# Linyou/Ced-NeRF

Hardware: AMD Instinct MI355X
Metric: samples_per_sec (render_image_test, 800x800 D-NeRF lego-shaped synthetic) (higher is better)
Workload: dtype f32 (MLP GEMMs: split-fp16 MFMA, 22-bit operands, fp32 accumulate)

## Files before the change

### ced_nerf_amd/_lib.py

```python
from __future__ import annotations

import ctypes as C
import os
import subprocess
from typing import List, Optional

_PKG = os.path.dirname(os.path.abspath(__file__))
_ROOT = os.path.dirname(_PKG)
LIB_PATH = os.environ.get("CED_NERF_LIB", os.path.join(_PKG, "libcednerf_hip.so"))
SOURCES = ["runtime.hip", "march.hip", "composite.hip", "field.hip", "hash.hip", "field_half.hip", "field_mixed.hip", "field_move.hip", "field_jacobian.hip", "field_density_gradient.hip", "field_time_max.hip", "field_level_set.hip", "surface.hip", "frame_loop.hip", "frame.hip", "image.hip", "march_all.hip", "occgrid.hip",
           "raygen.hip", "wgrad.hip", "pixels.hip", "accel.hip", "linear.hip", "mlp.hip", "train_glue.hip", "losses.hip",
           "metrics.hip", "train_batch.hip", "importance.hip", "bake.hip", "mesh.hip"]
MLP_F32, MLP_F16X2, MLP_F16, MLP_F32_HEAD16X2 = 0, 1, 2, 3
MLP_PRECISIONS = {"f32": MLP_F32, "f16x2": MLP_F16X2, "f16": MLP_F16, "f32+h16x2": MLP_F32_HEAD16X2}
HIPCC_FLAGS = ["--offload-arch=gfx950", "-O3", "-ffp-contract=off", "-fno-slp-vectorize", "-fPIC", "-shared", "-std=c++17"]
PER_SOURCE_FLAGS = {"field_half.hip": ["-mllvm", "-amdgpu-sched-strategy=max-memory-clause"]}
MAX_LEVELS = 16


class HashDesc(C.Structure):
    _fields_ = [
        ("n_levels", C.c_int32), ("table_dtype", C.c_int32), ("temporal", C.c_int32), ("reserved", C.c_int32),
        ("scale", C.c_float * MAX_LEVELS), ("res", C.c_uint32 * MAX_LEVELS), ("offset", C.c_uint32 * MAX_LEVELS),
        ("size", C.c_uint32 * MAX_LEVELS), ("hashed", C.c_uint32 * MAX_LEVELS),
        ("table", C.c_void_p), ("total_entries", C.c_uint64),
    ]


class FieldDesc(C.Structure):
    _fields_ = [
        ("aabb", C.c_float * 6), ("moving_step", C.c_float), ("use_div_offsets", C.c_int32),
        ("time_mode", C.c_int32), ("mlp_precision", C.c_int32), ("max_workgroups", C.c_int32),
        ("packed_weights", C.c_void_p), ("packed_floats", C.c_uint64),
        ("hash", HashDesc),
    ]


class FrameTrace(C.Structure):
    _fields_ = [
        ("capacity", C.c_int32), ("n_iters", C.c_int32),
        ("field_begin", C.POINTER(C.c_void_p)), ("field_end", C.POINTER(C.c_void_p)),
        ("iter_alive", C.POINTER(C.c_int64)), ("iter_n_samples", C.POINTER(C.c_int64)),
        ("iter_samples", C.POINTER(C.c_int64)), ("field_stamps", C.c_void_p),
    ]


EXCHANGE_FN = C.CFUNCTYPE(C.c_int, C.c_void_p, C.c_void_p, C.c_int32, C.c_int32, C.c_void_p)


class ShardExchange(C.Structure):
    _fields_ = [
        ("global_rays_per_frame", C.c_int64), ("local_rays", C.c_void_p), ("counts", C.c_void_p),
        ("reduce", EXCHANGE_FN), ("user", C.c_void_p),
    ]


_vp, _i64, _i32, _f = C.c_void_p, C.c_int64, C.c_int32, C.c_float

PROTOTYPES = {
    "ced_version": (C.c_int, []),
    "ced_last_error_string": (C.c_char_p, []),
    "ced_set_option": (C.c_int, [C.c_char_p, C.c_int]),
    "ced_packed_weight_floats": (_i64, [C.c_int, C.c_int]),
    "ced_pack_field_weights": (C.c_int, [C.c_int, C.c_int] + [_vp] * 10),
    "ced_packed_weight_words": (_i64, [C.c_int, C.c_int, C.c_int]),
    "ced_pack_field_weights_half": (C.c_int, [C.c_int, C.c_int, C.c_int] + [_vp] * 10),
    "ced_pack_field_weights_half_for": (C.c_int, [C.c_int] * 5 + [_vp] * 10),
    "ced_pack_field_weights_mixed": (C.c_int, [C.c_int, C.c_int] + [_vp] * 10),
    "ced_ray_aabb_intersect": (C.c_int, [_i64, _vp, _vp, _i32, _vp, _f, _f, _f, _vp, _vp, _vp, _vp]),
    "ced_sort_intersections": (C.c_int, [_i64, _i32, _vp, _vp, _vp, _vp, _vp]),
    "ced_traverse_grids": (C.c_int, [_i64, _vp, _vp, _vp, _i32, _i32, _vp, _vp, _vp, _f, _f, _i32, _vp, _vp, _vp, _vp,
                                     _i32, _vp, _vp, _vp, _vp, _vp, _vp, _vp, _vp]),
    "ced_host_skip_march": (_f, [_f, _f, _f, _f]),
    "ced_occupancy_accel_bytes": (_i64, [_i32, _i32]),
    "ced_build_occupancy_accel": (C.c_int, [_vp, _i32, _i32, _vp, _i64, _vp]),
    "ced_host_build_occupancy_accel": (C.c_int, [_vp, _i32, _i32, _vp]),
    "ced_host_count_steps": (_i32, [C.POINTER(C.c_float), _f, _f, _i32, C.POINTER(C.c_float)]),
    "ced_host_march_frame": (C.c_int, [_i64, _vp, _vp, _vp, _i32, _i32, _vp, _vp, _f, _f, _f, _i32, _vp, _vp, _vp, _vp, _i32, _i32,
                                       _i32, _vp, _vp, _vp, _vp]),
    "ced_hash_encode": (C.c_int, [C.POINTER(HashDesc), _i64, _vp, _vp, _vp, _vp]),
    "ced_hash_encode_backward": (C.c_int, [C.POINTER(HashDesc), _i64, _vp, _vp, _vp, _vp, _i32, _vp]),
    "ced_hash_encode_backward_temporal": (C.c_int, [C.POINTER(HashDesc), _i64, _vp, _vp, _vp, _vp, _vp]),
    "ced_field_forward": (C.c_int, [C.POINTER(FieldDesc), _i64, _vp, _vp, _vp, _vp, _vp, _vp, _vp]),
    "ced_field_forward_rays": (C.c_int, [C.POINTER(FieldDesc), _i64, _vp, _vp, _vp, _vp, _vp, _vp, _vp, _i32, _i32,
                                         _vp, _vp, _vp]),
    "ced_field_move": (C.c_int, [C.POINTER(FieldDesc), _i64, _vp, _vp, _vp, _vp, _vp, _vp, _vp]),
    "ced_field_move_rays": (C.c_int, [C.POINTER(FieldDesc), _i64, _vp, _vp, _vp, _vp, _vp, _vp, _vp, _i32, _vp, _vp, _vp]),
    "ced_field_move_inverse": (C.c_int, [C.POINTER(FieldDesc), _i64, _vp, _vp, _vp, _i32, _f, _vp, _vp, _vp, _vp]),
    "ced_field_track": (C.c_int, [C.POINTER(FieldDesc), _i64, _i64, _vp, _vp, _vp, _i32, _f, _vp, _vp, _vp, _vp]),
    "ced_field_move_jacobian": (C.c_int, [C.POINTER(FieldDesc), _i64, _vp, _vp, _vp, _vp, _vp]),
    "ced_field_density_gradient": (C.c_int, [C.POINTER(FieldDesc), _i64, _vp, _vp, _vp, _vp, _vp, _vp, _vp]),
    "ced_field_density_gradient_rays": (C.c_int, [C.POINTER(FieldDesc), _i64, _vp, _vp, _vp, _vp, _vp, _vp, _vp, _i32, _vp, _vp,
                                                  _vp, _vp, _vp]),
    "ced_field_density_time_max": (C.c_int, [C.POINTER(FieldDesc), _i64, _vp, _i32, _i32, _vp, _vp, _vp]),
    "ced_surface_first_crossing": (C.c_int, [_i64, _vp, _vp, _vp, _vp, _f, _vp, _vp, _vp, _vp]),
    "ced_field_level_set": (C.c_int, [C.POINTER(FieldDesc), _i64, _vp, _vp, _vp, _vp, _vp, _i32, _f, _i32, _f, _vp, _vp, _vp, _vp,
                                      _vp, _vp, _vp]),
    "ced_field_velocity": (C.c_int, [C.POINTER(FieldDesc), _i64, _vp, _vp, _vp, _vp, _vp, _vp]),
    "ced_field_velocity_rays": (C.c_int, [C.POINTER(FieldDesc), _i64, _vp, _vp, _vp, _vp, _vp, _vp, _vp, _i32, _vp, _vp, _vp, _vp]),
    "ced_field_move_inverse_newton": (C.c_int, [C.POINTER(FieldDesc), _i64, _vp, _vp, _vp, _i32, _f, _vp, _vp, _vp, _vp]),
    "ced_field_track_newton": (C.c_int, [C.POINTER(FieldDesc), _i64, _i64, _vp, _vp, _vp, _i32, _f, _vp, _vp, _vp, _vp]),
    "ced_field_rgb": (C.c_int, [C.POINTER(FieldDesc), _i64, _vp, _vp, _i32, _vp, _vp]),
    "ced_field_rgb_bcast": (C.c_int, [C.POINTER(FieldDesc), _i64, _i32, _vp, _vp, _i32, _vp, _vp]),
    "ced_bake_workspace_bytes": (_i64, [_i64]),
    "ced_bake_candidates": (C.c_int, [_i32, C.POINTER(C.c_float), _f, _i64, _i64, _vp, _vp, _i32, _i32, _i64, _vp, _vp, _vp,
                                      _vp, _i64, _vp]),
    "ced_bake_select": (C.c_int, [_i64, _vp, _vp, _vp, _vp, _f, _i64, _vp, _vp, _vp, _vp, _vp, _vp, _i64, _vp]),
    "ced_mesh_workspace_bytes": (_i64, [_i32]),
    "ced_mesh_vertices": (C.c_int, [_i32, C.POINTER(C.c_float), _f, _vp, _f, _i64, _vp, _vp, _vp, _vp, _vp, _i64, _vp]),
    "ced_mesh_faces": (C.c_int, [_i32, _vp, _f, _vp, _i64, _i64, _vp, _vp, _vp, _i64, _vp]),
    "ced_render_weights": (C.c_int, [_i64, _vp, _vp, _vp, _vp, _vp, _vp, _vp, _vp, _vp]),
    "ced_accumulate_along_rays": (C.c_int, [_i64, _vp, _vp, _vp, _i32, _vp, _vp]),
    "ced_reduce_along_rays": (C.c_int, [_i64, _vp, _vp, _i32, _vp, _i32, _i64, _i32, _vp, _vp, _vp]),
    "ced_visibility_mask": (C.c_int, [_i64, _vp, _vp, _vp, _vp, _f, _f, _vp, _vp]),
    "ced_composite_prefix": (C.c_int, [_i64, _vp, _vp, _vp, _vp, _vp, _vp, _vp, _vp, _vp]),
    "ced_composite_backward": (C.c_int, [_i64, _vp, _vp, _vp, _vp, _vp, _vp, _vp, _vp, _vp, _vp, _vp]),
    "ced_distortion_workspace_bytes": (_i64, [_i64, _i64, _i32]),
    "ced_distortion_loss": (C.c_int, [_i64, _i64] + [_vp] * 10),
    "ced_distortion_loss_density": (C.c_int, [_i64, _i64] + [_vp] * 10),
    "ced_ssim_workspace_bytes": (_i64, [_i64, _i64, _i64, _i64, _i32, _i32]),
    "ced_ssim": (C.c_int, [_i64, _i64, _i64, _i64, _vp, C.POINTER(_i64), _vp, C.POINTER(_i64), C.c_double, C.c_double,
                           C.c_double, _i32, C.POINTER(C.c_float), _i32, C.POINTER(C.c_float), _i32, _vp, _vp, _vp, _vp,
                           _vp, _vp]),
    "ced_frame_to_rgb8": (C.c_int, [_i32, _i32, _vp, _i32, _vp, _vp]),
    "ced_flow_to_rgb8": (C.c_int, [_i32, _i32, _vp, _f, _i32, _vp, _vp]),
    "ced_depth_to_u8": (C.c_int, [_i32, _i32, _vp, _i32, _vp, _vp, _vp]),
    "ced_scatter_pixels": (C.c_int, [_i64, _vp, _i32, _vp, _i32, _vp, _i32, _vp, _i64, _vp, _vp, _vp, _vp, _i32, _i32, _vp]),
    "ced_linear": (C.c_int, [_i64, _vp, _i32, _vp, _i32, _i32, _i32, _i32, _i32, _vp, _vp, _vp]),
    "ced_weight_grad_workspace_bytes": (_i64, [_i64, _i32, _i32]),
    "ced_weight_grad": (C.c_int, [_i64, _vp, _i32, _vp, _i32, _vp, _vp, _i64, _vp]),
    "ced_composite_step": (C.c_int, [_i64, _vp, _vp, _vp, _vp, _vp, _vp, _vp, _vp, _f, _i32, _vp, _vp, _vp]),
    "ced_composite_test": (C.c_int, [_i64, _vp, _vp, _vp, _vp, _vp, _vp, _f, _f, _vp, _vp, _vp, _vp]),
    "ced_finalize_pixels": (C.c_int, [_i64, _vp, _vp, _vp, _vp, _vp]),
    "ced_occ_cell_points": (C.c_int, [_i64, _vp, _vp, _i32, C.POINTER(C.c_float), _vp, _vp]),
    "ced_occ_ema_update": (C.c_int, [_i64, _vp, _vp, _f, _f, _vp, _vp, _i64, _vp]),
    "ced_occ_time_slices_workspace_bytes": (_i64, [_i32, _i32, _i32]),
    "ced_occ_time_slices": (C.c_int, [_i64, _vp, _vp, _i32, _f, _f, _i32, _i32, _vp, _i32, _vp, _vp, _i64, _vp]),
    "ced_generate_rays_pinhole": (C.c_int, [_i32, _i32, _f, _f, _f, _f, C.POINTER(C.c_float), _i32, _vp, _vp, _vp, _vp]),
    "ced_generate_rays_hypercam": (C.c_int, [_i32, _i32, C.POINTER(C.c_float), C.POINTER(C.c_float), _f, _f, _f, _f, _f,
                                             C.POINTER(C.c_float), C.POINTER(C.c_float), _vp, _vp, _vp]),
    "ced_sample_training_batch": (C.c_int, [_i32] * 5 + [_vp] * 3 + [_i64, C.c_uint64, _i64, _i32, _i32] + [_vp] * 7),
    "ced_importance_batch_workspace_bytes": (_i64, [_i64, _i64, _i64]),
    "ced_sample_importance_batch": (C.c_int, [_i32] * 5 + [_vp] * 4 + [_i32, _i64, _i64, C.c_uint64, _i64, _i32] + [_vp] * 8
                                    + [_i64, _vp]),
    "ced_temporal_median_u8": (C.c_int, [_i32] * 4 + [_vp] * 3),
    "ced_isg_weights": (C.c_int, [_i32] * 4 + [_vp, _vp, _f, _vp, _vp]),
    "ced_ist_weights": (C.c_int, [_i32] * 4 + [_vp, _f, _i32, _vp, _vp]),
    "ced_render_image_test_workspace_bytes": (_i64, [_i64, _i32, _i32, _f, _i32]),
    "ced_render_image_test": (C.c_int, [C.POINTER(FieldDesc), _i64, _vp, _vp, _vp, _i32, _i32, _vp, _vp, _f, _f, _f, _f, _f,
                                        _i32, _vp, _i32, _vp, _vp, _vp, _vp, _vp, _i64, _vp, C.POINTER(_i64),
                                        C.POINTER(FrameTrace), _vp, _vp]),
    "ced_render_frames_test_workspace_bytes": (_i64, [_i32, _i64, _i32, _i32, _f, _i32]),
    "ced_render_frames_test": (C.c_int, [C.POINTER(FieldDesc), _i32, _i64, _vp, _vp, _vp, _i32, _i32, _vp, _vp, _f, _f, _f, _f,
                                         _f, _i32, _vp, _vp, _vp, _vp, _vp, _vp, _i64, _vp, C.POINTER(_i64),
                                         C.POINTER(FrameTrace), _vp, _vp]),
    "ced_render_frames_test_sharded_workspace_bytes": (_i64, [_i32, _i64, _i64, _i32, _i32, _f, _i32]),
    "ced_render_frames_test_iterations": (_i32, [_f, _i32]),
    "ced_render_frames_test_host_bytes": (_i64, [_f, _i32]),
    "ced_render_frames_test_sharded": (C.c_int, [C.POINTER(FieldDesc), _i32, _i64, _vp, _vp, _vp, _i32, _i32, _vp, _vp, _f, _f, _f,
                                                 _f, _f, _i32, _vp, _vp, _vp, _vp, _vp, _vp, _i64, _vp, C.POINTER(_i64),
                                                 C.POINTER(FrameTrace), _vp, _vp, C.POINTER(ShardExchange)]),
    "ced_wall_clock_khz": (_i64, []),
    "ced_mlp_chain": (C.c_int, [_i64, _i32, _i32, _vp, C.POINTER(_i32), C.POINTER(_vp), C.POINTER(_vp), C.POINTER(_vp), _i32, _vp]),
    "ced_march_all": (C.c_int, [_i64, _vp, _vp, _vp, _i32, _i32, _vp, _vp, _vp, _f, _f, _f, _vp, _vp, _vp, _i32, _vp, _vp, _vp,
                                _vp, _i64, _vp, _vp]),
    "ced_render_image_workspace_bytes": (_i64, [_i64, _i64]),
    "ced_render_image": (C.c_int, [C.POINTER(FieldDesc), _i64, _vp, _vp, _i64, _vp, _vp, _vp, _f, _f, _vp, _i32, _vp, _vp, _vp,
                                   _vp, _vp, _vp, _i64, _vp, C.POINTER(_i64), _vp, _vp]),
    "ced_mlp_backward_dw_workspace_bytes": (_i64, [_i64, _i32, C.POINTER(_i32)]),
    "ced_mlp_backward_dw": (C.c_int, [_i64, _i32, _vp, C.POINTER(_i32), C.POINTER(_vp), C.POINTER(_vp), _vp, _vp, _vp, _i64, _vp]),
    "ced_train_inputs": (C.c_int, [_i64] + [_vp] * 13),
    "ced_train_warp": (C.c_int, [_i64, _vp, _vp, _i32, _i32, _f, C.POINTER(C.c_float), _vp, _vp, _vp, _vp]),
    "ced_train_warp_backward": (C.c_int, [_i64, _vp, _vp, _i32, _i32, _f, C.POINTER(C.c_float), _vp, _vp, _vp, _vp]),
    "ced_train_head_in": (C.c_int, [_i64] + [_vp] * 6),
    "ced_train_head_in_backward": (C.c_int, [_i64] + [_vp] * 6),
    "ced_render_image_gather": (C.c_int, [_i64, _i64, _i64, _vp, _i64, _vp, _i64, _vp, _vp, _vp, _vp, _vp, _vp, _vp, _vp, _vp]),
}


def _includes(path: str, seen=None) -> List[str]:
    import re
    seen = set() if seen is None else seen
    if path in seen or not os.path.exists(path):
        return []
    seen.add(path)
    out = [path]
    for inc in re.findall(r'^\s*#\s*include\s+"([^"]+)"', open(path).read(), flags=re.M):
        out += _includes(os.path.normpath(os.path.join(os.path.dirname(path), inc)), seen)
    return out


def build(force: bool = False, verbose: bool = False, extra_flags: Optional[List[str]] = None) -> str:
    from concurrent.futures import ThreadPoolExecutor
    srcs = [os.path.join(_PKG, "csrc", s) for s in SOURCES]
    hipcc = os.environ.get("HIPCC", "hipcc")
    flags = [f for f in HIPCC_FLAGS if f != "-shared"] + list(extra_flags or [])
    obj_dir = os.path.join(_ROOT, "build", "obj")
    os.makedirs(obj_dir, exist_ok=True)
    stamp = os.path.join(obj_dir, "flags.txt")
    flag_text = " ".join([hipcc] + flags + [f"{k}:{' '.join(v)}" for k, v in sorted(PER_SOURCE_FLAGS.items())])
    if not os.path.exists(stamp) or open(stamp).read() != flag_text:
        force = True
    jobs, objs = [], []
    for src in srcs:
        obj = os.path.join(obj_dir, os.path.basename(src) + ".o")
        objs.append(obj)
        deps = _includes(src)
        if force or not os.path.exists(obj) or any(os.path.getmtime(obj) < os.path.getmtime(d) for d in deps):
            jobs.append([hipcc] + flags + PER_SOURCE_FLAGS.get(os.path.basename(src), []) + ["-c", src, "-o", obj])
    if not jobs and os.path.exists(LIB_PATH) and all(os.path.getmtime(LIB_PATH) >= os.path.getmtime(o) for o in objs):
        return LIB_PATH

    def run(cmd):
        if verbose:
            print(" ".join(cmd), flush=True)
        subprocess.check_call(cmd)

    workers = max(1, min(len(jobs), int(os.environ.get("CED_BUILD_JOBS", str(min(os.cpu_count() or 1, 8))))))
    if jobs:
        with ThreadPoolExecutor(max_workers=workers) as pool:
            list(pool.map(run, jobs))
    run([hipcc, "--offload-arch=gfx950", "-shared", "-fPIC", "-o", LIB_PATH] + objs)
    from . import _k32_gate
    _, bad = _k32_gate.check(LIB_PATH)
    if bad:
        os.remove(LIB_PATH)
        raise RuntimeError("K = 32 residency gate failed (ced_nerf_amd/_k32_gate.py): "
                           + "; ".join(f"{k}: {v}" for k, v in sorted(bad.items())))
    with open(stamp, "w") as f:
        f.write(flag_text)
    return LIB_PATH


_lib: Optional[C.CDLL] = None


def lib() -> C.CDLL:
    global _lib
    if _lib is None:
        if not os.path.exists(LIB_PATH):
            raise RuntimeError(
                f"{LIB_PATH} not found: build the HIP extension first (python -c 'import __graft_entry__ as g; "
                "g.build()'); ced_nerf_amd has no CPU fallback")
        handle = C.CDLL(LIB_PATH)
        for name, (res, args) in PROTOTYPES.items():
            fn = getattr(handle, name)
            fn.restype = res
            fn.argtypes = args
        _lib = handle
        for item in filter(None, os.environ.get("CED_OPTIONS", "").split(",")):
            key, _, value = item.partition("=")
            if handle.ced_set_option(key.strip().encode(), int(value)) != 0:
                raise RuntimeError(f"CED_OPTIONS: {handle.ced_last_error_string().decode()}")
    return _lib


def check(rc: int, what: str = "") -> None:
    if rc != 0:
        msg = lib().ced_last_error_string()
        raise RuntimeError(f"libcednerf_hip {what} failed (code {rc}): {msg.decode() if msg else ''}")


def header_symbols() -> List[str]:
    import re
    text = open(os.path.join(_ROOT, "include", "cednerf_hip.h")).read()
    text = re.sub(r"/\*.*?\*/", "", text, flags=re.S)
    return sorted(set(re.findall(r"\b(ced_[a-z0-9_]+)\s*\(", text)))
```

### ced_nerf_amd/csrc/accel.hip

```cpp
#include <algorithm>
#include <vector>

#include "ced_common.hpp"
#include "march_accel.hpp"

namespace ced {

constexpr int kDistCap = 15;

__global__ __launch_bounds__(64) void brick_any_kernel(const uint8_t *__restrict__ binaries, int res, int nb,
                                                       uint8_t *__restrict__ any)
{
    const int idx = blockIdx.x;
    const int bz = idx % nb, by = (idx / nb) % nb, bx = (idx / (nb * nb)) % nb, lvl = idx / (nb * nb * nb);
    const uint8_t *g = binaries + (size_t)lvl * res * res * res;
    const int x = bx * kBrick + (threadIdx.x >> 3), y = by * kBrick + (threadIdx.x & 7);
    uint8_t acc = 0;
    if (x < res && y < res)
        for (int z = bz * kBrick; z < min((bz + 1) * kBrick, res); ++z) acc |= g[((size_t)x * res + y) * res + z];
    const unsigned long long any_lane = __ballot(acc != 0);
    if (threadIdx.x == 0) any[idx] = any_lane ? 0 : 255;
}

__global__ __launch_bounds__(1024) void brick_dist_lds_kernel(uint8_t *__restrict__ dist, int nb)
{
    extern __shared__ uint8_t sm[];
    const int n = nb * nb * nb;
    uint8_t *cur = sm, *nxt = sm + n;
    uint8_t *level = dist + (size_t)blockIdx.x * n;
    for (int i = threadIdx.x; i < n; i += blockDim.x) cur[i] = level[i];
    __syncthreads();
    for (int r = 1; r <= kDistCap; ++r) {
        for (int i = threadIdx.x; i < n; i += blockDim.x) {
            uint8_t v = cur[i];
            if (v == 255) {
                const int bz = i % nb, by = (i / nb) % nb, bx = i / (nb * nb);
                bool reach = false;
                for (int x = max(bx - 1, 0); x <= min(bx + 1, nb - 1); ++x)
                    for (int y = max(by - 1, 0); y <= min(by + 1, nb - 1); ++y)
                        for (int z = max(bz - 1, 0); z <= min(bz + 1, nb - 1); ++z) reach |= cur[(x * nb + y) * nb + z] != 255;
                if (reach) v = (uint8_t)r;
            }
            nxt[i] = v;
        }
        __syncthreads();
        uint8_t *t = cur; cur = nxt; nxt = t;
    }
    for (int i = threadIdx.x; i < n; i += blockDim.x) level[i] = cur[i] == 255 ? (uint8_t)(kDistCap + 1) : cur[i];
}

__global__ __launch_bounds__(256) void brick_dist_round_kernel(const uint8_t *__restrict__ src, uint8_t *__restrict__ dst,
                                                               int n_levels, int nb, int r, int final_round)
{
    const int64_t idx = (int64_t)blockIdx.x * blockDim.x + threadIdx.x;
    const int64_t n = (int64_t)nb * nb * nb;
    if (idx >= n * n_levels) return;
    const int i = (int)(idx % n);
    const uint8_t *lv = src + (idx / n) * n;
    uint8_t v = lv[i];
    if (v == 255) {
        const int bz = i % nb, by = (i / nb) % nb, bx = i / (nb * nb);
        bool reach = false;
        for (int x = max(bx - 1, 0); x <= min(bx + 1, nb - 1); ++x)
            for (int y = max(by - 1, 0); y <= min(by + 1, nb - 1); ++y)
                for (int z = max(bz - 1, 0); z <= min(bz + 1, nb - 1); ++z) reach |= lv[(x * nb + y) * nb + z] != 255;
        if (reach) v = (uint8_t)r;
    }
    if (final_round && v == 255) v = (uint8_t)(kDistCap + 1);
    dst[idx] = v;
}

constexpr int kCellCap = 15;

__global__ __launch_bounds__(256) void cell_dist_z_kernel(const uint8_t *__restrict__ binaries, int n_levels, int res,
                                                          uint8_t *__restrict__ out)
{
    const int64_t col = (int64_t)blockIdx.x * blockDim.x + threadIdx.x;
    if (col >= (int64_t)n_levels * res * res) return;
    const uint8_t *g = binaries + col * res;
    uint8_t *o = out + col * res;
    int dmin = kCellCap + 1;
    for (int z = 0; z < res; ++z) {
        dmin = g[z] ? 0 : min(dmin + 1, kCellCap + 1);
        o[z] = (uint8_t)dmin;
    }
    dmin = kCellCap + 1;
    for (int z = res - 1; z >= 0; --z) {
        dmin = g[z] ? 0 : min(dmin + 1, kCellCap + 1);
        o[z] = (uint8_t)min((int)o[z], dmin);
    }
}

__global__ __launch_bounds__(256) void cell_dist_axis_kernel(const uint8_t *__restrict__ src, uint8_t *__restrict__ dst,
                                                             int n_levels, int res, int axis)
{
    const int64_t idx = (int64_t)blockIdx.x * blockDim.x + threadIdx.x;
    const int64_t n = (int64_t)res * res * res;
    if (idx >= n * n_levels) return;
    const int i = (int)(idx % n);
    const int z = i % res, y = (i / res) % res, x = i / (res * res);
    const int pos = axis == 0 ? x : y;
    const int64_t stride = axis == 0 ? (int64_t)res * res : res;
    int best = src[idx];
    for (int k = 1; k < best && k <= kCellCap; ++k) {
        if (pos - k >= 0) best = min(best, max(k, (int)src[idx - k * stride]));
        if (pos + k < res) best = min(best, max(k, (int)src[idx + k * stride]));
    }
    (void)z;
    dst[idx] = (uint8_t)best;
}

__global__ __launch_bounds__(256) void cell_dist_combine_kernel(uint8_t *__restrict__ cdist, const uint8_t *__restrict__ bdist,
                                                                int n_levels, int res, int nb)
{
    const int64_t idx = (int64_t)blockIdx.x * blockDim.x + threadIdx.x;
    const int64_t n = (int64_t)res * res * res;
    if (idx >= n * n_levels) return;
    int v = cdist[idx];
    if (v > kCellCap) {
        const int i = (int)(idx % n);
        const int z = i % res, y = (i / res) % res, x = i / (res * res);
        const int R = bdist[((idx / n) * nb + (x >> kBrickShift)) * nb * nb + (int64_t)(y >> kBrickShift) * nb + (z >> kBrickShift)];
        const int bound = R >= 1 ? (R - 1) * kBrick + 1 : 0;
        v = max(kCellCap + 1, bound);
        cdist[idx] = (uint8_t)min(v, 255);
    }
}

static inline int64_t align256(int64_t x) { return (x + 255) & ~(int64_t)255; }

AccelSpec accel_view(const void *accel, int n_grids, int res, bool with_cells)
{
    const int nb = (res + kBrick - 1) / kBrick;
    const uint8_t *base = (const uint8_t *)accel;
    return AccelSpec{ base, nb, with_cells ? base + align256(2 * (int64_t)n_grids * nb * nb * nb) : nullptr };
}

int build_brick_accel(const uint8_t *binaries, int n_grids, int res, uint8_t *dist, uint8_t *scratch, hipStream_t stream)
{
    const int nb = (res + kBrick - 1) / kBrick;
    const int n_bricks = n_grids * nb * nb * nb;
    hipLaunchKernelGGL(brick_any_kernel, dim3(n_bricks), dim3(64), 0, stream, binaries, res, nb, dist);
    if (nb <= 32) {
        hipLaunchKernelGGL(brick_dist_lds_kernel, dim3(n_grids), dim3(1024), (size_t)2 * nb * nb * nb, stream, dist, nb);
    } else {
        uint8_t *src = dist, *dst = scratch;
        for (int r = 1; r <= kDistCap; ++r) {
            hipLaunchKernelGGL(brick_dist_round_kernel, dim3((n_bricks + 255) / 256), dim3(256), 0, stream, src, dst, n_grids,
                               nb, r, r == kDistCap ? 1 : 0);
            uint8_t *t = src; src = dst; dst = t;
        }
        if (src != dist && hipMemcpyAsync(dist, src, (size_t)n_bricks, hipMemcpyDeviceToDevice, stream) != hipSuccess)
            return check_launch("build_occupancy_accel (copy)");
    }
    return check_launch("build_occupancy_accel (bricks)");
}

int build_full_accel(const uint8_t *binaries, int n_grids, int res, uint8_t *accel, hipStream_t stream)
{
    const int64_t nb = (res + kBrick - 1) / kBrick;
    const int64_t n_bricks = n_grids * nb * nb * nb, n_cells = (int64_t)n_grids * res * res * res;
    uint8_t *bdist = accel, *cdist = accel + align256(2 * n_bricks), *cscr = cdist + n_cells;
    int rc = build_brick_accel(binaries, n_grids, res, bdist, bdist + n_bricks, stream);
    if (rc) return rc;
    const dim3 blk(256), grd((unsigned)((n_cells + 255) / 256));
    hipLaunchKernelGGL(cell_dist_z_kernel, dim3((unsigned)(((int64_t)n_grids * res * res + 255) / 256)), blk, 0, stream, binaries,
                       n_grids, res, cdist);
    hipLaunchKernelGGL(cell_dist_axis_kernel, grd, blk, 0, stream, cdist, cscr, n_grids, res, 1);
    hipLaunchKernelGGL(cell_dist_axis_kernel, grd, blk, 0, stream, cscr, cdist, n_grids, res, 0);
    hipLaunchKernelGGL(cell_dist_combine_kernel, grd, blk, 0, stream, cdist, bdist, n_grids, res, (int)nb);
    return check_launch("build_occupancy_accel (cells)");
}

static void host_build_bricks(const uint8_t *binaries, int n_grids, int res, uint8_t *dist)
{
    const int nb = (res + kBrick - 1) / kBrick;
    const size_t n = (size_t)nb * nb * nb;
    for (int lvl = 0; lvl < n_grids; ++lvl) {
        const uint8_t *g = binaries + (size_t)lvl * res * res * res;
        uint8_t *lv = dist + lvl * n;
        for (size_t i = 0; i < n; ++i) lv[i] = 255;
        for (int x = 0; x < res; ++x)
            for (int y = 0; y < res; ++y)
                for (int z = 0; z < res; ++z)
                    if (g[((size_t)x * res + y) * res + z]) lv[((size_t)(x / kBrick) * nb + y / kBrick) * nb + z / kBrick] = 0;
        std::vector<uint8_t> nxt(n);
        for (int r = 1; r <= kDistCap; ++r) {
            for (size_t i = 0; i < n; ++i) {
                uint8_t v = lv[i];
                if (v == 255) {
                    const int bz = (int)(i % nb), by = (int)((i / nb) % nb), bx = (int)(i / ((size_t)nb * nb));
                    bool reach = false;
                    for (int x = bx > 0 ? bx - 1 : 0; x <= (bx + 1 < nb ? bx + 1 : nb - 1); ++x)
                        for (int y = by > 0 ? by - 1 : 0; y <= (by + 1 < nb ? by + 1 : nb - 1); ++y)
                            for (int z = bz > 0 ? bz - 1 : 0; z <= (bz + 1 < nb ? bz + 1 : nb - 1); ++z)
                                reach |= lv[((size_t)x * nb + y) * nb + z] != 255;
                    if (reach) v = (uint8_t)r;
                }
                nxt[i] = v;
            }
            for (size_t i = 0; i < n; ++i) lv[i] = nxt[i];
        }
        for (size_t i = 0; i < n; ++i)
            if (lv[i] == 255) lv[i] = (uint8_t)(kDistCap + 1);
    }
}

static void host_build_cells(const uint8_t *binaries, int n_grids, int res, const uint8_t *bdist, uint8_t *cdist)
{
    const int nb = (res + kBrick - 1) / kBrick;
    const int64_t n = (int64_t)res * res * res;
    std::vector<uint8_t> tmp((size_t)n);
    for (int lvl = 0; lvl < n_grids; ++lvl) {
        const uint8_t *g = binaries + lvl * n;
        uint8_t *out = cdist + lvl * n;
        for (int64_t col = 0; col < (int64_t)res * res; ++col) {
            int dmin = kCellCap + 1;
            for (int z = 0; z < res; ++z) { dmin = g[col * res + z] ? 0 : std::min(dmin + 1, kCellCap + 1); out[col * res + z] = (uint8_t)dmin; }
            dmin = kCellCap + 1;
            for (int z = res - 1; z >= 0; --z) {
                dmin = g[col * res + z] ? 0 : std::min(dmin + 1, kCellCap + 1);
                out[col * res + z] = (uint8_t)std::min((int)out[col * res + z], dmin);
            }
        }
        for (int axis = 1; axis >= 0; --axis) {
            const int64_t stride = axis == 0 ? (int64_t)res * res : res;
            for (int64_t row = 0; row < (int64_t)res * res; ++row) {
                const int pos = axis == 0 ? (int)(row / res) : (int)(row % res);
                const uint8_t *src = out + row * res;
                uint8_t *best = tmp.data() + row * res;
                for (int z = 0; z < res; ++z) best[z] = src[z];
                for (int k = 1; k <= kCellCap; ++k) {
                    for (int side = -1; side <= 1; side += 2) {
                        if (pos + side * k < 0 || pos + side * k >= res) continue;
                        const uint8_t *nbr = src + side * k * stride;
                        for (int z = 0; z < res; ++z) best[z] = std::min(best[z], std::max((uint8_t)k, nbr[z]));
                    }
                }
            }
            for (int64_t i = 0; i < n; ++i) out[i] = tmp[(size_t)i];
        }
        for (int64_t i = 0; i < n; ++i) {
            int v = out[i];
            if (v > kCellCap) {
                const int z = (int)(i % res), y = (int)((i / res) % res), x = (int)(i / ((int64_t)res * res));
                const int R = bdist[(((size_t)lvl * nb + (x >> kBrickShift)) * nb + (y >> kBrickShift)) * nb + (z >> kBrickShift)];
                const int bound = R >= 1 ? (R - 1) * kBrick + 1 : 0;
                out[i] = (uint8_t)std::min(std::max(kCellCap + 1, bound), 255);
            }
        }
    }
}

}

extern "C" int64_t ced_occupancy_accel_bytes(int32_t n_grids, int32_t res)
{
    if (n_grids < 1 || res < 1 || res > 1024) return -1;
    const int64_t nb = (res + ced::kBrick - 1) / ced::kBrick;
    return ced::align256(2 * (int64_t)n_grids * nb * nb * nb) + 2 * (int64_t)n_grids * res * res * res;
}

extern "C" int ced_build_occupancy_accel(const uint8_t *binaries, int32_t n_grids, int32_t res, void *accel,
                                         int64_t accel_bytes, void *stream)
{
    CED_REQUIRE(binaries && accel, "build_occupancy_accel: null pointer");
    const int64_t need = ced_occupancy_accel_bytes(n_grids, res);
    CED_REQUIRE(need > 0 && accel_bytes >= need, "build_occupancy_accel: bad sizes (need %lld bytes, got %lld)",
                (long long)need, (long long)accel_bytes);
    return ced::build_full_accel(binaries, n_grids, res, (uint8_t *)accel, (hipStream_t)stream);
}

extern "C" int ced_host_build_occupancy_accel(const uint8_t *binaries_host, int32_t n_grids, int32_t res,
                                              uint8_t *accel_host)
{
    CED_REQUIRE(binaries_host && accel_host && n_grids >= 1 && res >= 1 && res <= 1024, "host_build_occupancy_accel: bad arguments");
    const int64_t nb = (res + ced::kBrick - 1) / ced::kBrick;
    ced::host_build_bricks(binaries_host, n_grids, res, accel_host);
    ced::host_build_cells(binaries_host, n_grids, res, accel_host, accel_host + ced::align256(2 * (int64_t)n_grids * nb * nb * nb));
    return CED_OK;
}

extern "C" int32_t ced_host_count_steps(float *x, float d, float tau, int32_t kcap, float *prev)
{
    return ced::count_steps(*x, d, tau, kcap, *prev);
}

extern "C" int ced_host_march_frame(int64_t n_rays, const float *rays_o, const float *rays_d, const uint8_t *binaries,
                                    int32_t n_grids, int32_t res, const float *aabbs, const float *near_planes,
                                    float far_plane, float step_size, float cone_angle, int32_t limit,
                                    const float *t_sorted, const int64_t *t_indices, const uint8_t *hits,
                                    const uint8_t *accel_host, int32_t accel_mode, int32_t use_lattice, int32_t walk,
                                    int32_t *counts, float *t_starts, float *t_ends, float *t_term)
{
    CED_REQUIRE(n_rays >= 0 && n_grids >= 1 && res >= 1 && limit >= 1, "host_march_frame: bad sizes");
    CED_REQUIRE(rays_o && rays_d && binaries && aabbs && near_planes && t_sorted && t_indices && hits && counts &&
                    t_starts && t_ends && t_term, "host_march_frame: null pointer");
    CED_REQUIRE(accel_mode >= 0 && accel_mode <= 2 && (accel_mode == 0 || accel_host), "host_march_frame: accel_mode 0 (none), 1 (bricks), 2 (cells)");
    CED_REQUIRE(walk >= 0 && walk <= 3, "host_march_frame: walk 0..3");
    float lattice[256];
    if (use_lattice) ced::build_lattice(near_planes[0], step_size, lattice);
    const ced::GridSpec G{ binaries, aabbs, n_grids, res, step_size, cone_angle, limit,
                           (use_lattice && walk != 3 && cone_angle == 0.0f && step_size > 0.0f) ? lattice : nullptr };
    ced::AccelSpec S{ nullptr, (res + ced::kBrick - 1) / ced::kBrick, nullptr };
    if (accel_mode) S = ced::accel_view(accel_host, n_grids, res, accel_mode == 2);
    for (int64_t r = 0; r < n_rays; ++r) {
        const float o[3] = { rays_o[3 * r], rays_o[3 * r + 1], rays_o[3 * r + 2] };
        const float d[3] = { rays_d[3 * r], rays_d[3 * r + 1], rays_d[3 * r + 2] };
        float *t0 = t_starts + r * limit, *t1 = t_ends + r * limit;
        auto emit = [&](int i, float a, float b) { t0[i] = a; t1[i] = b; };
        const float *ts = t_sorted + r * 2 * n_grids;
        const int64_t *ti = t_indices + r * 2 * n_grids;
        const uint8_t *hr = hits + r * n_grids;
        const float near = near_planes[r];
        float &tt = t_term[r];
        if (walk == 3)
            counts[r] = ced::traverse_ray(G, o, d, near, far_plane, ts, ti, hr, emit, tt);
        else if (n_grids == 1)
            counts[r] = walk == 1 ? ced::traverse_ray_frame<ced::kFrameLook, true, true>(G, S, true, o, d, near, far_plane, ts, ti, hr, emit, tt)
                                  : ced::traverse_ray_frame<ced::kFrameLook, true, false>(G, S, walk != 0, o, d, near, far_plane, ts, ti, hr, emit, tt);
        else
            counts[r] = walk == 1 ? ced::traverse_ray_frame<ced::kFrameLook, false, true>(G, S, true, o, d, near, far_plane, ts, ti, hr, emit, tt)
                                  : ced::traverse_ray_frame<ced::kFrameLook, false, false>(G, S, walk != 0, o, d, near, far_plane, ts, ti, hr, emit, tt);
    }
    return CED_OK;
}
```

### ced_nerf_amd/csrc/frame.hip

```cpp
#include "ced_common.hpp"
#include "composite_core.hpp"
#include "field_args.hpp"
#include "frame_loop.hpp"
#include "march_accel.hpp"
#include "march_diag.hpp"
#include "march_pack.hpp"

namespace ced {

int build_brick_accel(const uint8_t *binaries, int n_grids, int res, uint8_t *dist, uint8_t *scratch, hipStream_t stream);
AccelSpec accel_view(const void *accel, int n_grids, int res, bool with_cells);

__global__ __launch_bounds__(256) void frame_times_kernel(int64_t n_rays, int rays_per_frame,
                                                          const float *__restrict__ frame_times, float *__restrict__ ts_ray)
{
    const int64_t r = (int64_t)blockIdx.x * blockDim.x + threadIdx.x;
    if (r < n_rays) ts_ray[r] = frame_times[r / rays_per_frame];
}

__global__ __launch_bounds__(256) void frame_prep_kernel(int64_t n_rays, const float *__restrict__ rays_o,
                                                         const float *__restrict__ rays_d, int m,
                                                         const float *__restrict__ aabbs, float near_plane,
                                                         float *__restrict__ t_sorted, uint8_t *__restrict__ t_indices,
                                                         uint8_t *__restrict__ hits, float *__restrict__ near_planes,
                                                         float *__restrict__ sh_ray, float *__restrict__ rgb,
                                                         float *__restrict__ opacity, float *__restrict__ depth)
{
    int64_t r = (int64_t)blockIdx.x * blockDim.x + threadIdx.x;
    if (r >= n_rays) return;
    const float o[3] = { rays_o[3 * r], rays_o[3 * r + 1], rays_o[3 * r + 2] };
    const float inv_d[3] = { 1.0f / rays_d[3 * r], 1.0f / rays_d[3 * r + 1], 1.0f / rays_d[3 * r + 2] };
    float ev[2 * kMaxGrids];
    int id[2 * kMaxGrids];
    for (int a = 0; a < m; ++a) {
        float t0 = __builtin_inff(), t1 = __builtin_inff();
        bool hit = slab_test(o, inv_d, aabbs + 6 * a, t0, t1);
        if (!hit) { t0 = __builtin_inff(); t1 = __builtin_inff(); }
        hits[r * m + a] = hit ? 1 : 0;
        ev[a] = t0; id[a] = a;
        ev[m + a] = t1; id[m + a] = m + a;
    }
    if (m > 1) {
        for (int i = 1; i < 2 * m; ++i) {
            float v = ev[i];
            int k = id[i], j = i - 1;
            while (j >= 0 && ev[j] > v) { ev[j + 1] = ev[j]; id[j + 1] = id[j]; --j; }
            ev[j + 1] = v; id[j + 1] = k;
        }
    }
    for (int i = 0; i < 2 * m; ++i) {
        t_sorted[r * 2 * m + i] = ev[i];
        t_indices[r * 2 * m + i] = (uint8_t)id[i];
    }
    near_planes[r] = near_plane;
    reset_ray(rays_d, r, sh_ray, rgb, opacity, depth);
}

__global__ __launch_bounds__(256) void frame_prep_single_kernel(int64_t n_rays, const float *__restrict__ rays_d,
                                                                float near_plane, float *__restrict__ near_planes,
                                                                float *__restrict__ sh_ray, float *__restrict__ rgb,
                                                                float *__restrict__ opacity, float *__restrict__ depth)
{
    int64_t r = (int64_t)blockIdx.x * blockDim.x + threadIdx.x;
    if (r >= n_rays) return;
    near_planes[r] = near_plane;
    reset_ray(rays_d, r, sh_ray, rgb, opacity, depth);
}

struct MarchArgs {
    const float *rays_o, *rays_d;
    GridSpec grid;
    AccelSpec accel;
    float *near_planes;
    float far_plane;
    const int32_t *alive;
    int n_frames, rays_per_frame;
    const float *t_sorted;
    const uint8_t *t_indices;
    const uint8_t *hits;
    float *t_starts, *t_ends;
    int32_t *ray_idx;
    int32_t *packed;
    int32_t *cand;
};

constexpr int kCullThreads = 256;
static_assert(kSlotAlign % kCullThreads == 0, "a culling workgroup's slots belong to one frame");
template <bool SINGLE>
__global__ __launch_bounds__(kCullThreads) void march_cull_kernel(MarchArgs A, IterPlan *__restrict__ plan)
{
    const IterPlan &P = *plan;
    const int64_t total = P.total_slots;
    const int m = SINGLE ? 1 : A.grid.n_grids, res = A.grid.res;
    for (int64_t s0 = (int64_t)blockIdx.x * kCullThreads; s0 < total; s0 += (int64_t)gridDim.x * kCullThreads) {
        const int f = frame_of_slot(P, A.n_frames, s0);
        if (f < 0) continue;
        const int64_t idx = s0 + threadIdx.x - P.slot_base[f];
        const bool active = idx < P.count[f];
        const int64_t r = (int64_t)f * A.rays_per_frame + (active ? idx : 0);
        bool cand = false;
        if (active) {
            float o[3], d[3];
#pragma unroll
            for (int a = 0; a < 3; ++a) { o[a] = A.rays_o[3 * r + a]; d[a] = A.rays_d[3 * r + a]; }
            const float near = A.near_planes[r];
            const float inv_d[3] = { 1.0f / d[0], 1.0f / d[1], 1.0f / d[2] };
            const float *ts_row = SINGLE ? nullptr : A.t_sorted + r * 2 * m;
            const uint8_t *ti_row = SINGLE ? nullptr : A.t_indices + r * 2 * m;
            const uint8_t *hit_row = SINGLE ? nullptr : A.hits + r * m;
            for (int i = 0; i < 2 * m - 1 && !cand; ++i) {
                int lvl;
                float seg_a, seg_b;
                if (!decode_segment<SINGLE>(A.grid, o, inv_d, ts_row, ti_row, hit_row, i, lvl, seg_a, seg_b)) continue;
                const float t0 = fmaxf(seg_a, near), t1 = fminf(seg_b, A.far_plane);
                if (t0 >= t1) continue;
                float t_stop, cells;
                cand = !coarse_advance(A.accel, lvl, res, A.grid.aabbs + 6 * lvl, o, d, t0, t1, t_stop, cells);
            }
            if (!cand) { A.packed[2 * r] = 0; A.packed[2 * r + 1] = 0; }
        }
        const int slot = workgroup_append<kCullThreads / 64, 0>(
            cand, nullptr, [&](int run, const int *) { return run > 0 ? atomicAdd(&plan->n_cand, run) : 0; });
        if (cand) A.cand[slot] = (int32_t)r;
        __syncthreads();
    }
}

constexpr int kCandLanes = 64;
template <bool SINGLE, bool CAND, bool FIRST>
__global__ __launch_bounds__(kMarchThreads, (SINGLE && !CAND) ? 4 : 3) void march_frame_kernel(MarchArgs A, IterPlan *__restrict__ plan)
{
    static_assert(!CAND || FIRST, "the candidate list belongs to the first iteration");
    constexpr int kWaves = kMarchThreads / 64;
    constexpr int kPerGroup = CAND ? kWaves * kCandLanes : kMarchThreads;
    const IterPlan &P = *plan;
    const int64_t total = CAND ? (int64_t)P.n_cand : (int64_t)P.total_slots;
    const int lane = threadIdx.x & 63, wave = threadIdx.x >> 6;
    for (int64_t s0 = (int64_t)blockIdx.x * kPerGroup; s0 < total; s0 += (int64_t)gridDim.x * kPerGroup) {
        int f = 0;
        bool active;
        int64_t r = 0;
        if constexpr (CAND) {
            const int64_t slot = s0 + wave * kCandLanes + lane;
            active = lane < kCandLanes && slot < total;
            if (active) { r = A.cand[slot]; f = (int)(r / A.rays_per_frame); }
        } else {
            f = frame_of_slot(P, A.n_frames, s0);
            if (f < 0) continue;
            const int64_t idx = s0 + threadIdx.x - P.slot_base[f];
            active = idx < P.count[f];
            const int64_t first = (int64_t)f * A.rays_per_frame;
            r = active ? (A.alive ? (int64_t)A.alive[first + idx] : first + idx) : 0;
        }
        const int limit = P.limit[f];
        GridSpec grid = A.grid;
        grid.limit = limit;
        const int m = grid.n_grids;
        float o[3] = { 0.0f, 0.0f, 0.0f }, d[3] = { 0.0f, 0.0f, 1.0f };
        float near = 0.0f;
        const auto walk = [&](auto first, auto &&emit) {
            if constexpr (decltype(first)::value) {
#pragma unroll
                for (int a = 0; a < 3; ++a) { o[a] = A.rays_o[3 * r + a]; d[a] = A.rays_d[3 * r + a]; }
                near = A.near_planes[r];
            }
            float t_term = 0.0f;
            const int n = traverse_ray_frame<kFrameLook, SINGLE, FIRST>(
                grid, A.accel, FIRST, o, d, near, A.far_plane,
                SINGLE ? nullptr : A.t_sorted + r * 2 * m, SINGLE ? (const uint8_t *)nullptr : A.t_indices + r * 2 * m,
                SINGLE ? nullptr : A.hits + r * m, emit, t_term);
            if constexpr (decltype(first)::value) A.near_planes[r] = t_term;
            return n;
        };
        float *p0 = nullptr, *p1 = nullptr;
        int32_t *pr = nullptr;
        CED_DIAG_TICK(0);
        pack_ray_samples<kWaves>(
            active, grid, walk,
            [&](int run) {
                return (long long)atomicAdd(reinterpret_cast<unsigned long long *>(&plan->total_samples), (unsigned long long)run);
            },
            [&](int64_t start, int n) {
                A.packed[2 * r] = (int32_t)start;
                A.packed[2 * r + 1] = n;
                p0 = A.t_starts + start; p1 = A.t_ends + start; pr = A.ray_idx + start;
                return true;
            },
            [&](int i, float t0, float t1) { p0[i] = t0; p1[i] = t1; pr[i] = (int32_t)r; });
        CED_DIAG_TICK(7);
        __syncthreads();
    }
#ifdef CED_MARCH_DIAG
    ced_diag_flush();
#endif
}

__global__ __launch_bounds__(kCompositeThreads) void frame_composite_kernel(
    IterPlan *plan, int n_frames, int rays_per_frame, const int32_t *__restrict__ alive_list,
    int32_t *__restrict__ next_list, const int32_t *__restrict__ packed, const float *__restrict__ t0,
    const float *__restrict__ t1, const float *__restrict__ sig, const float *__restrict__ rgbs, float *__restrict__ rgb,
    float *__restrict__ opacity, float *__restrict__ depth, float opc_thres)
{
    const IterPlan &P = *plan;
    const int64_t total = P.total_slots;
    for (int64_t s0 = (int64_t)blockIdx.x * kCompositeThreads; s0 < total; s0 += (int64_t)gridDim.x * kCompositeThreads) {
        const int f = frame_of_slot(P, n_frames, s0);
        if (f < 0) continue;
        const int limit = P.limit[f];
        const int64_t idx = s0 + threadIdx.x - P.slot_base[f];
        const bool active = idx < P.count[f];
        const int64_t first = (int64_t)f * rays_per_frame;
        const int64_t r = active ? (alive_list ? (int64_t)alive_list[first + idx] : first + idx) : 0;
        int cnt = 0;
        bool alive = false;
        if (active) {
            cnt = packed[2 * r + 1];
            const float op = composite_ray(r, packed[2 * r], cnt, t0, t1, sig, rgbs, rgb, opacity, depth);
            alive = !P.last[f] && survives(op, cnt, limit, opc_thres);
        }
        const int slot = workgroup_append<kCompositeThreads / 64, 1>(alive, &cnt, [&](int run, const int *samples) {
            const unsigned long long add = (unsigned long long)run + ((unsigned long long)samples[0] << 32);
            return add != 0 ? (int)(atomicAdd(&plan->next[f], add) & 0xffffffffull) : 0;
        });
        if (alive) next_list[first + slot] = (int32_t)r;
        __syncthreads();
    }
}

__global__ __launch_bounds__(64) void frame_pack_counts_kernel(const IterPlan *__restrict__ plan, int n_frames,
                                                               int64_t *__restrict__ row)
{
    const int f = threadIdx.x;
    if (f >= n_frames) return;
    const unsigned long long nx = __hip_atomic_load(&plan->next[f], __ATOMIC_RELAXED, __HIP_MEMORY_SCOPE_AGENT);
    const bool finished = plan->last[f] || plan->gcount[f] == 0 || plan->count[f] == 0;
    row[f] = finished ? 0 : (int64_t)(nx & 0xffffffffull);
}

struct FrameWorkspace {
    float *t_sorted; uint8_t *t_indices; uint8_t *hits; float *near; int32_t *packed;
    int32_t *alive_a, *alive_b;
    IterPlan *plans;
    float *lattice;
    float *ts_ray;
    float *t0, *t1; int32_t *ridx; float *sigma, *rgbs;
    uint8_t *accel;
    float *sh_ray;
    size_t bytes;
};

static inline int min_samples_of(float cone_angle) { return cone_angle == 0.0f ? 1 : 4; }
static inline int max_iterations(int max_samples, int min_samples) { return (max_samples + min_samples - 1) / min_samples; }

static inline int64_t sample_capacity(int n_frames, int64_t rays_per_frame, int min_samples, int64_t global_rays)
{
    int64_t per = rays_per_frame * min_samples;
    if (global_rays > rays_per_frame) {
        const int64_t worst = rays_per_frame * 64 < global_rays ? rays_per_frame * 64 : global_rays;
        if (worst > per) per = worst;
    }
    return per * n_frames;
}

static FrameWorkspace carve(void *base, int64_t n, int m, int64_t cap, int max_iters, int res, bool per_ray_times = false)
{
    FrameWorkspace w{};
    Carver c{ (char *)base };
    w.t_sorted = c.take<float>((size_t)n * 2 * m);
    w.t_indices = c.take<uint8_t>((size_t)n * 2 * m);
    w.hits = c.take<uint8_t>((size_t)n * m);
    w.near = c.take<float>((size_t)n);
    w.packed = c.take<int32_t>((size_t)n * 2);
    w.alive_a = c.take<int32_t>((size_t)n);
    w.alive_b = c.take<int32_t>((size_t)n);
    w.plans = c.take<IterPlan>((size_t)max_iters + 2);
    w.lattice = c.take<float>(256);
    w.ts_ray = c.take<float>(per_ray_times ? (size_t)n : 0);
    w.t0 = c.take<float>((size_t)cap);
    w.t1 = c.take<float>((size_t)cap);
    w.ridx = c.take<int32_t>((size_t)cap);
    w.sigma = c.take<float>((size_t)cap);
    w.rgbs = c.take<float>((size_t)cap * 3);
    const int64_t nbk = (res + kBrick - 1) / kBrick;
    w.accel = c.take<uint8_t>((size_t)(2 * m * nbk * nbk * nbk));
    w.sh_ray = c.take<float>((size_t)n * 3);
    w.bytes = c.off;
    return w;
}

struct FrameCall {
    const char *who;
    const ced_field_desc *field;
    int n_frames;
    int64_t rays_per_frame, workspace_bytes;
    const float *rays_o, *rays_d, *aabbs, *timestamps, *frame_times, *bkgd;
    const uint8_t *binaries;
    const void *accel;
    int32_t n_grids, res, max_samples, t_per_ray;
    float near_plane, far_plane, step_size, cone_angle, early_stop_eps;
    float *rgb, *opacity, *depth;
    void *workspace, *field_stream, *stream;
    int64_t *host_stats, *total_samples_out;
    ced_frame_trace *trace;
    const ced_shard_exchange *xch;
};

static int render_frames_impl(const FrameCall &c)
{
    hipStream_t stream = (hipStream_t)c.stream;
    hipStream_t fstream = c.field_stream ? (hipStream_t)c.field_stream : stream;
    const bool split = fstream != stream;
    constexpr int kMaxDevices = 64;
    static thread_local hipEvent_t ev_to_field[kMaxDevices] = {}, ev_from_field[kMaxDevices] = {};
    int dev = 0;
    if (split) {
        if (hipGetDevice(&dev) != hipSuccess || dev < 0 || dev >= kMaxDevices) return check_launch("render_image_test (device)");
        if (!ev_to_field[dev] &&
            (hipEventCreateWithFlags(&ev_to_field[dev], hipEventDisableTiming) != hipSuccess ||
             hipEventCreateWithFlags(&ev_from_field[dev], hipEventDisableTiming) != hipSuccess))
            return check_launch("render_image_test (event create)");
    }
    const int64_t n_rays = (int64_t)c.n_frames * c.rays_per_frame;
    CED_REQUIRE(c.field != nullptr, "%s: null field descriptor", c.who);
    CED_REQUIRE(c.n_frames >= 1 && c.n_frames <= kMaxFrames, "%s: n_frames must be 1..%d", c.who, kMaxFrames);
    CED_REQUIRE(c.rays_per_frame >= 0 && c.n_grids >= 1 && c.n_grids <= kMaxGrids && c.res >= 1 && c.res <= 1024, "%s: bad sizes", c.who);
    CED_REQUIRE(n_rays < (1ll << 31) / 4, "%s: too many rays for 32-bit sample indices", c.who);
    CED_REQUIRE(c.max_samples >= 0, "%s: max_samples < 0", c.who);
    if (c.total_samples_out)
        for (int f = 0; f < c.n_frames; ++f) c.total_samples_out[f] = 0;
    if (c.trace) c.trace->n_iters = 0;
    if (n_rays == 0) return CED_OK;
    CED_REQUIRE(c.rays_o && c.rays_d && c.binaries && c.aabbs && (c.timestamps || c.frame_times) && c.rgb && c.opacity && c.depth &&
                    c.workspace && c.host_stats,
                "%s: null pointer", c.who);
    const int min_samples = min_samples_of(c.cone_angle);
    const int64_t cap = sample_capacity(c.n_frames, c.rays_per_frame, min_samples, c.xch ? c.xch->global_rays_per_frame : 0);
    CED_REQUIRE(cap < (1ll << 31) - 64, "%s: too many samples per iteration for 32-bit sample indices", c.who);
    const int max_iters = max_iterations(c.max_samples, min_samples);
    FrameWorkspace W = carve(c.workspace, n_rays, c.n_grids, cap, max_iters, c.res, c.frame_times != nullptr);
    CED_REQUIRE((int64_t)W.bytes <= c.workspace_bytes, "%s: workspace too small (%lld < %lld bytes)", c.who,
                (long long)c.workspace_bytes, (long long)W.bytes);
    if (c.xch) {
        CED_REQUIRE(c.xch->reduce && c.xch->counts && c.xch->global_rays_per_frame >= c.rays_per_frame &&
                        c.xch->global_rays_per_frame < (1ll << 31),
                    "%s: bad ced_shard_exchange (reduce / counts NULL, or global_rays_per_frame < rays_per_frame)", c.who);
        CED_REQUIRE(!c.field_stream || c.field_stream == c.stream, "%s: a sharded call takes no separate field stream", c.who);
    }
    const dim3 blk(256), grd((unsigned)((n_rays + 255) / 256));

    if (c.n_grids == 1)
        hipLaunchKernelGGL(frame_prep_single_kernel, grd, blk, 0, stream, n_rays, c.rays_d, c.near_plane, W.near, W.sh_ray, c.rgb,
                           c.opacity, c.depth);
    else
        hipLaunchKernelGGL(frame_prep_kernel, grd, blk, 0, stream, n_rays, c.rays_o, c.rays_d, (int)c.n_grids, c.aabbs, c.near_plane,
                           W.t_sorted, W.t_indices, W.hits, W.near, W.sh_ray, c.rgb, c.opacity, c.depth);
    if (c.frame_times)
        hipLaunchKernelGGL(frame_times_kernel, grd, blk, 0, stream, n_rays, (int)c.rays_per_frame, c.frame_times, W.ts_ray);
    const int nb = (c.res + kBrick - 1) / kBrick;
    AccelSpec acc;
    if (c.accel) {
        acc = accel_view(c.accel, c.n_grids, c.res, true);
    } else {
        int rc = build_brick_accel(c.binaries, c.n_grids, c.res, W.accel, W.accel + (size_t)c.n_grids * nb * nb * nb, stream);
        if (rc) return rc;
        acc = AccelSpec{ W.accel, nb, nullptr };
    }
    const bool use_lattice = c.cone_angle == 0.0f && c.step_size > 0.0f && c.near_plane >= 0.0f;
    if (use_lattice) build_lattice(c.near_plane, c.step_size, reinterpret_cast<float *>(c.host_stats + kHostLatticeWord));
    FrameLoop L{ ScheduleArgs{ W.plans, -1, c.n_frames, (int)c.rays_per_frame, min_samples, (int)c.max_samples,
                               (long long *)c.host_stats, 0, c.xch ? c.xch->local_rays : nullptr,
                               c.xch ? c.xch->counts : nullptr, c.xch ? c.xch->global_rays_per_frame : 0,
                               c.xch ? (long long *)c.host_stats + kHostIterWord : nullptr },
                 W.alive_a, W.alive_b, max_iters, c.who };
    L.begin(stream, use_lattice ? W.lattice : nullptr, (unsigned long long *)(c.trace ? c.trace->field_stamps : nullptr),
            (c.trace && c.trace->field_stamps) ? (int)c.trace->capacity : 0);
    int rc = check_launch("render_image_test (prep)");
    if (rc) return rc;

    const float opc_thres = (float)(1.0 - (double)c.early_stop_eps);
    for (; L.it < L.max_iters; ++L.it) {
        bool stop = false;
        rc = L.next(stop);
        if (rc) return rc;
        if (stop) break;
        const int it = L.it;
        IterPlan *plan = L.plan();
        const int32_t *cur_list = L.cur_list();
        int32_t *next_list = L.next_list();

        const int64_t slot_bound = L.alive_bound + (int64_t)c.n_frames * kSlotAlign;
        MarchArgs M{ c.rays_o, c.rays_d,
                     GridSpec{ c.binaries, c.aabbs, c.n_grids, c.res, c.step_size, c.cone_angle, 0, use_lattice ? W.lattice : nullptr },
                     acc, W.near, c.far_plane, cur_list, c.n_frames, (int)c.rays_per_frame, W.t_sorted, W.t_indices, W.hits,
                     W.t0, W.t1, W.ridx, W.packed, W.alive_b };
        int64_t mgrid = (slot_bound + kMarchThreads - 1) / kMarchThreads;
        if (mgrid > 8192) mgrid = 8192;
        const dim3 mblk(kMarchThreads);
        const int two_pass_opt = g_march_two_pass;
        const bool two_pass = two_pass_opt < 0 ? c.n_grids > 1 : two_pass_opt != 0;
        with_bool(c.n_grids == 1, [&](auto single) {
            constexpr bool kSingle = decltype(single)::value;
            if (it == 0 && acc.bdist && two_pass) {
                int64_t kgrid = (slot_bound + kCullThreads - 1) / kCullThreads;
                if (kgrid > 8192) kgrid = 8192;
                if (mgrid > 4096) mgrid = 4096;
                hipLaunchKernelGGL(march_cull_kernel<kSingle>, dim3((unsigned)kgrid), dim3(kCullThreads), 0, stream, M, plan);
                hipLaunchKernelGGL((march_frame_kernel<kSingle, true, true>), dim3((unsigned)mgrid), mblk, 0, stream, M, plan);
            } else if (it == 0) {
                hipLaunchKernelGGL((march_frame_kernel<kSingle, false, true>), dim3((unsigned)mgrid), mblk, 0, stream, M, plan);
            } else {
                hipLaunchKernelGGL((march_frame_kernel<kSingle, false, false>), dim3((unsigned)mgrid), mblk, 0, stream, M, plan);
            }
        });
        rc = check_launch("render_image_test (march)");
        if (rc) return rc;

        FieldArgs F{};
        F.n = cap;
        F.n_dev = &plan->total_samples;
        F.rays_o = c.rays_o; F.rays_d = c.rays_d; F.ray_idx32 = W.ridx;
        F.sh_ray = g_frame_sh_per_ray ? W.sh_ray : nullptr;
        F.t0 = W.t0; F.t1 = W.t1;
        F.timestamps = c.frame_times ? W.ts_ray : c.timestamps;
        F.rays_mode = 1; F.t_per_ray = (c.frame_times || c.t_per_ray) ? 1 : 0; F.want_rgb = 1;
        F.rgb = W.rgbs; F.sigma = W.sigma; F.geo = nullptr;
        if (c.trace && c.trace->field_stamps && it < c.trace->capacity)
            F.stamp = reinterpret_cast<unsigned long long *>(c.trace->field_stamps) + 2 * it;
        if (split) {
            (void)hipEventRecord(ev_to_field[dev], stream);
            (void)hipStreamWaitEvent(fstream, ev_to_field[dev], 0);
        }
        if (c.trace && it < c.trace->capacity && c.trace->field_begin)
            (void)hipEventRecord((hipEvent_t)c.trace->field_begin[it], fstream);
        rc = launch_field(c.field, F, (void *)fstream);
        if (rc) return rc;
        if (c.trace && it < c.trace->capacity && c.trace->field_end)
            (void)hipEventRecord((hipEvent_t)c.trace->field_end[it], fstream);
        if (split) {
            (void)hipEventRecord(ev_from_field[dev], fstream);
            (void)hipStreamWaitEvent(stream, ev_from_field[dev], 0);
        }

        int64_t cgrid = (slot_bound + kCompositeThreads - 1) / kCompositeThreads;
        if (cgrid > 4096) cgrid = 4096;
        hipLaunchKernelGGL(frame_composite_kernel, dim3((unsigned)cgrid), dim3(kCompositeThreads), 0, stream,
                           plan, c.n_frames, (int)c.rays_per_frame, cur_list, next_list, W.packed, W.t0, W.t1, W.sigma, W.rgbs,
                           c.rgb, c.opacity, c.depth, opc_thres);
        int64_t *xrow = nullptr;
        if (c.xch) {
            xrow = c.xch->counts + (int64_t)it * c.n_frames;
            hipLaunchKernelGGL(frame_pack_counts_kernel, dim3(1), dim3(64), 0, stream, plan, c.n_frames, xrow);
            rc = check_launch("render_image_test (pack counts)");
            if (rc) return rc;
            const int xrc = c.xch->reduce(c.xch->user, xrow, c.n_frames, it, (void *)stream);
            if (xrc != 0) {
                set_error("%s: the exchange step of iteration %d failed (code %d)", c.who, it, xrc);
                (void)hipStreamSynchronize(stream);
                return CED_E_LAUNCH;
            }
        }
        L.schedule(stream);
        rc = check_launch("render_image_test (composite / schedule)");
        if (rc) return rc;
    }
    rc = ced_finalize_pixels(n_rays, c.bkgd, c.rgb, c.opacity, c.depth, stream);
    if (rc) return rc;
    std::vector<IterPlan> plans;
    int n_iters = 0;
    rc = L.finish(stream, "render_image_test (read-back)", plans, n_iters);
    if (rc) return rc;
    int64_t total[kMaxFrames] = { 0 };
    for (int k = 0; k < n_iters; ++k) {
        const IterPlan &P = plans[k];
        int64_t alive_total = 0, samples_it = 0;
        int max_limit = 0;
        for (int f = 0; f < c.n_frames; ++f) {
            alive_total += P.count[f];
            samples_it += (int64_t)(P.next[f] >> 32);
            total[f] += (int64_t)(P.next[f] >> 32);
            if (P.count[f] > 0 && P.limit[f] > max_limit) max_limit = P.limit[f];
        }
        if (c.trace && k < c.trace->capacity) {
            if (c.trace->iter_alive) c.trace->iter_alive[k] = alive_total;
            if (c.trace->iter_n_samples) c.trace->iter_n_samples[k] = max_limit;
            if (c.trace->iter_samples) c.trace->iter_samples[k] = samples_it;
        }
    }
    if (c.trace) c.trace->n_iters = n_iters;
    if (c.total_samples_out)
        for (int f = 0; f < c.n_frames; ++f) c.total_samples_out[f] = total[f];
    return CED_OK;
}

}

extern "C" int64_t ced_render_image_test_workspace_bytes(int64_t n_rays, int32_t n_grids, int32_t res,
                                                         float cone_angle, int32_t max_samples)
{
    if (n_rays < 0 || n_grids < 1 || n_grids > ced::kMaxGrids || res < 1 || res > 1024 || max_samples < 0) return -1;
    const int ms = ced::min_samples_of(cone_angle);
    return (int64_t)ced::carve(nullptr, n_rays, n_grids, n_rays * ms, ced::max_iterations(max_samples, ms), res).bytes;
}

extern "C" int ced_render_image_test(const ced_field_desc *field, int64_t n_rays, const float *rays_o,
                                     const float *rays_d, const uint8_t *binaries, int32_t n_grids, int32_t res,
                                     const float *aabbs, const void *accel, float near_plane, float far_plane,
                                     float step_size, float cone_angle, float early_stop_eps, int32_t max_samples,
                                     const float *timestamps, int32_t t_per_ray, const float *bkgd, float *rgb,
                                     float *opacity, float *depth, void *workspace, int64_t workspace_bytes,
                                     int64_t *host_stats, int64_t *total_samples_out, ced_frame_trace *trace,
                                     void *field_stream_, void *stream_)
{
    ced::FrameCall c{};
    c.who = "render_image_test"; c.field = field; c.n_frames = 1; c.rays_per_frame = n_rays; c.rays_o = rays_o; c.rays_d = rays_d;
    c.binaries = binaries; c.n_grids = n_grids; c.res = res; c.aabbs = aabbs; c.accel = accel; c.near_plane = near_plane;
    c.far_plane = far_plane; c.step_size = step_size; c.cone_angle = cone_angle; c.early_stop_eps = early_stop_eps;
    c.max_samples = max_samples; c.timestamps = timestamps; c.t_per_ray = t_per_ray; c.frame_times = nullptr; c.bkgd = bkgd;
    c.rgb = rgb; c.opacity = opacity; c.depth = depth; c.workspace = workspace; c.workspace_bytes = workspace_bytes;
    c.host_stats = host_stats; c.total_samples_out = total_samples_out; c.trace = trace; c.field_stream = field_stream_;
    c.stream = stream_; c.xch = nullptr;
    return ced::render_frames_impl(c);
}

extern "C" int64_t ced_render_frames_test_workspace_bytes(int32_t n_frames, int64_t rays_per_frame, int32_t n_grids,
                                                          int32_t res, float cone_angle, int32_t max_samples)
{
    return ced_render_frames_test_sharded_workspace_bytes(n_frames, rays_per_frame, rays_per_frame, n_grids, res, cone_angle,
                                                          max_samples);
}

extern "C" int ced_render_frames_test(const ced_field_desc *field, int32_t n_frames, int64_t rays_per_frame,
                                      const float *rays_o, const float *rays_d, const uint8_t *binaries, int32_t n_grids,
                                      int32_t res, const float *aabbs, const void *accel, float near_plane,
                                      float far_plane, float step_size, float cone_angle, float early_stop_eps,
                                      int32_t max_samples, const float *frame_times, const float *bkgd, float *rgb,
                                      float *opacity, float *depth, void *workspace, int64_t workspace_bytes,
                                      int64_t *host_stats, int64_t *total_samples_out, ced_frame_trace *trace,
                                      void *field_stream_, void *stream_)
{
    CED_REQUIRE(frame_times != nullptr, "render_frames_test: null frame_times");
    ced::FrameCall c{};
    c.who = "render_frames_test"; c.field = field; c.n_frames = n_frames; c.rays_per_frame = rays_per_frame; c.rays_o = rays_o; c.rays_d = rays_d;
    c.binaries = binaries; c.n_grids = n_grids; c.res = res; c.aabbs = aabbs; c.accel = accel; c.near_plane = near_plane;
    c.far_plane = far_plane; c.step_size = step_size; c.cone_angle = cone_angle; c.early_stop_eps = early_stop_eps;
    c.max_samples = max_samples; c.timestamps = nullptr; c.t_per_ray = 0; c.frame_times = frame_times; c.bkgd = bkgd;
    c.rgb = rgb; c.opacity = opacity; c.depth = depth; c.workspace = workspace; c.workspace_bytes = workspace_bytes;
    c.host_stats = host_stats; c.total_samples_out = total_samples_out; c.trace = trace; c.field_stream = field_stream_;
    c.stream = stream_; c.xch = nullptr;
    return ced::render_frames_impl(c);
}

extern "C" int64_t ced_render_frames_test_sharded_workspace_bytes(int32_t n_frames, int64_t rays_per_frame,
                                                                  int64_t global_rays_per_frame, int32_t n_grids,
                                                                  int32_t res, float cone_angle, int32_t max_samples)
{
    if (n_frames < 1 || n_frames > ced::kMaxFrames || rays_per_frame < 0 || global_rays_per_frame < rays_per_frame ||
        n_grids < 1 || n_grids > ced::kMaxGrids || res < 1 || res > 1024 || max_samples < 0)
        return -1;
    const int64_t n_rays = (int64_t)n_frames * rays_per_frame;
    const int ms = ced::min_samples_of(cone_angle);
    return (int64_t)ced::carve(nullptr, n_rays, n_grids, ced::sample_capacity(n_frames, rays_per_frame, ms, global_rays_per_frame),
                               ced::max_iterations(max_samples, ms), res, true).bytes;
}

extern "C" int32_t ced_render_frames_test_iterations(float cone_angle, int32_t max_samples)
{
    if (max_samples < 0) return -1;
    return ced::max_iterations(max_samples, ced::min_samples_of(cone_angle));
}

extern "C" int64_t ced_render_frames_test_host_bytes(float cone_angle, int32_t max_samples)
{
    if (max_samples < 0) return -1;
    const int64_t iters = ced::max_iterations(max_samples, ced::min_samples_of(cone_angle));
    return (ced::kHostIterWord + 3 * (iters + 2)) * (int64_t)sizeof(int64_t);
}

extern "C" int ced_render_frames_test_sharded(const ced_field_desc *field, int32_t n_frames, int64_t rays_per_frame,
                                              const float *rays_o, const float *rays_d, const uint8_t *binaries,
                                              int32_t n_grids, int32_t res, const float *aabbs, const void *accel,
                                              float near_plane, float far_plane, float step_size, float cone_angle,
                                              float early_stop_eps, int32_t max_samples, const float *frame_times,
                                              const float *bkgd, float *rgb, float *opacity, float *depth, void *workspace,
                                              int64_t workspace_bytes, int64_t *host_stats, int64_t *total_samples_out,
                                              ced_frame_trace *trace, void *field_stream_, void *stream_,
                                              const ced_shard_exchange *exchange)
{
    CED_REQUIRE(frame_times != nullptr, "render_frames_test_sharded: null frame_times");
    ced::FrameCall c{};
    c.who = "render_frames_test_sharded"; c.field = field; c.n_frames = n_frames; c.rays_per_frame = rays_per_frame; c.rays_o = rays_o; c.rays_d = rays_d;
    c.binaries = binaries; c.n_grids = n_grids; c.res = res; c.aabbs = aabbs; c.accel = accel; c.near_plane = near_plane;
    c.far_plane = far_plane; c.step_size = step_size; c.cone_angle = cone_angle; c.early_stop_eps = early_stop_eps;
    c.max_samples = max_samples; c.timestamps = nullptr; c.t_per_ray = 0; c.frame_times = frame_times; c.bkgd = bkgd;
    c.rgb = rgb; c.opacity = opacity; c.depth = depth; c.workspace = workspace; c.workspace_bytes = workspace_bytes;
    c.host_stats = host_stats; c.total_samples_out = total_samples_out; c.trace = trace; c.field_stream = field_stream_;
    c.stream = stream_; c.xch = exchange;
    return ced::render_frames_impl(c);
}
```

### ced_nerf_amd/csrc/march_accel.hpp

```cpp
#pragma once
#include <cmath>

#include "march_core.hpp"

#if defined(CED_MARCH_DIAG) && defined(__HIP_DEVICE_COMPILE__)
__device__ void ced_diag_tick(int phase);
#define CED_DIAG_TICK(p) ced_diag_tick(p)
#else
#define CED_DIAG_TICK(p) ((void)0)
#endif

namespace ced {

constexpr int kBrickShift = 3;
constexpr int kLook = 8;
constexpr int kFrameLook = 4;
constexpr float kMinJumpCells = 3.0f;
constexpr int kCoarseRadius = 6;
static_assert((1 << kBrickShift) == kBrick, "brick size");

CED_HD int count_steps(float &x, float d, float tau, int kcap, float &prev)
{
    int k = 0;
    for (;;) {
        if (k >= kcap || !(x < tau)) break;
        const float x1 = x + d;
        Binade B;
        if (regular_binade(x, x1, d, B)) {
            const uint32_t X = B.X, INC = B.INC;
            uint32_t LIM = 0x1000000u;
            if (tau < bits_to_float(B.ex + (1u << 23))) LIM = (float_to_bits(tau) & 0x7fffffu) | 0x800000u;
            const uint32_t Q = LIM - X - 1u;
            uint32_t q = (uint32_t)((float)Q / (float)INC);
            if (q * INC > Q) --q;
            if ((q + 1u) * INC <= Q) ++q;
            uint32_t n = q + 1u;
            const uint32_t room = (uint32_t)(kcap - k);
            if (n > room) n = room;
            if (X + n * INC > 0xffffffu) --n;
            if (n >= 1u) {
                prev = B.term(n - 1u);
                x = B.term(n);
                k += (int)n;
                continue;
            }
        }
        prev = x;
        x = x1;
        ++k;
    }
    return k;
}

CED_HD float skip_march_lattice(const GridSpec &G, float t_last, float target)
{
    if (G.lattice && G.step_size > 0.0f && G.cone_angle == 0.0f) {
        const float A = target - G.step_size * 0.5f;
        const int e = (int)((float_to_bits(A) >> 23) & 0xffu);
        if ((float_to_bits(A) >> 31) == 0 && e >= 2 && e <= 254 && bits_to_float((uint32_t)(e - 1) << 23) > 4.0f * G.step_size) {
            const float first = G.lattice[e - 1];
            if (first > t_last && first < A - G.step_size) t_last = first;
        }
    }
    return skip_march(t_last, target, G.step_size, G.cone_angle);
}

CED_HD void build_lattice(float near, float step, float *lattice)
{
    for (int e = 0; e < 256; ++e) lattice[e] = bits_to_float(0x7fc00000u);
    if (!(step > 0.0f) || !(near >= 0.0f)) return;
    float t = near;
    for (int guard = 0; guard < 1024; ++guard) {
        const int e = (int)((float_to_bits(t) >> 23) & 0xffu);
        if (e >= 255 || t + step == t) break;
        if (!(lattice[e] == lattice[e])) lattice[e] = t;
        const float top = e == 0 ? bits_to_float(1u << 23) : bits_to_float((uint32_t)(e + 1) << 23);
        if (!(top < 3.0e38f)) break;
        float u = skip_march_const_step(t, top, step);
        int steps = 0;
        while ((int)((float_to_bits(u) >> 23) & 0xffu) == e && steps < 4) { const float v = u + step; if (v == u) return; u = v; ++steps; }
        if ((int)((float_to_bits(u) >> 23) & 0xffu) == e) return;
        t = u;
    }
}

struct AccelSpec {
    const uint8_t *bdist;
    int nb;
    const uint8_t *cdist;
};

CED_HD int empty_radius(const AccelSpec &S, int lvl, int res, int c0, int c1, int c2)
{
    if (S.cdist) return S.cdist[((size_t)lvl * res + c0) * res * res + (size_t)c1 * res + c2];
    const int R = S.bdist[(((size_t)lvl * S.nb + (c0 >> kBrickShift)) * S.nb + (c1 >> kBrickShift)) * S.nb + (c2 >> kBrickShift)];
    return R == 0 ? 0 : (R - 1) * kBrick + 1;
}

CED_HD bool coarse_advance(const AccelSpec &S, int lvl, int res, const float *__restrict__ ab, const float (&o)[3],
                           const float (&d)[3], float t_from, float t_to, float &t_stop, float &cells_skipped)
{
    const float resf = (float)res;
    float sc[3], g = 0.0f;
#pragma unroll
    for (int a = 0; a < 3; ++a) {
        sc[a] = resf / (ab[3 + a] - ab[a]);
        g = fmaxf(g, fabsf(d[a]) * sc[a]);
    }
    t_stop = t_from;
    cells_skipped = 0.0f;
    if (!(g > 0.0f) || !(g < 3.0e38f) || !(t_to - t_from < 3.0e38f)) return false;
    const float inv_g = 1.0f / g;
    float t = t_from;
    for (int guard = 0; guard < 8192; ++guard) {
        CED_DIAG_TICK(2);
        int c[3];
#pragma unroll
        for (int a = 0; a < 3; ++a) c[a] = clampi((int)((o[a] + d[a] * t - ab[a]) * sc[a]), 0, res - 1);
        const int D = empty_radius(S, lvl, res, c[0], c[1], c[2]);
        if (D < 4) { t_stop = t; cells_skipped = (t - t_from) * g; return false; }
        t += (float)(D - 3) * inv_g;
        if (t >= t_to) return true;
    }
    t_stop = t_from;
    return false;
}

struct Dda {
    float tdist[3], delta[3];
    int cur[3], stp[3], ovf[3];
    int safe_cell;
    bool done;
};

CED_HD void dda_setup_axis(Dda &D, int a, int res, const float *ab, const float (&o)[3], const float (&d)[3],
                           const float (&inv_d)[3], float this_tmin, float this_tmax)
{
    const float eps = 1e-6f;
    const float resf = (float)res;
    const float ts = this_tmin + eps, te = this_tmax - eps;
    const float ext = ab[3 + a] - ab[a];
    const float vox = ext / resf;
    const float ps = o[a] + d[a] * ts;
    const float pe = o[a] + d[a] * te;
    D.cur[a] = clampi((int)(((ps - ab[a]) / ext) * resf), 0, res - 1);
    const int fin = clampi((int)(((pe - ab[a]) / ext) * resf), 0, res - 1);
    const int idelta = d[a] > 0.0f ? 1 : 0;
    const float tm = ((ab[a] + (((float)(D.cur[a] + idelta) * vox) - ps)) * inv_d[a]) + this_tmin;
    const float stepf = (d[a] == 0.0f) ? 0.0f : (d[a] > 0.0f ? 1.0f : -1.0f);
    D.stp[a] = (int)stepf;
    const bool no_crossing = d[a] == 0.0f || (D.cur[a] == fin && tm < te);
    D.tdist[a] = no_crossing ? this_tmax : tm;
    D.delta[a] = (d[a] == 0.0f) ? this_tmax : (vox * inv_d[a]) * stepf;
    D.ovf[a] = fin + D.stp[a];
}

CED_HD void dda_begin(Dda &D, int res)
{
    D.safe_cell = (D.cur[0] * res + D.cur[1]) * res + D.cur[2];
    D.done = false;
}

template <int LOOK>
CED_HD unsigned look_ahead(Dda &D, int res, float this_tmax, float (&tt)[LOOK], int (&cellv)[LOOK])
{
    unsigned valid_mask = 0;
    int safe_cell = D.safe_cell;
    bool done = D.done;
#pragma unroll
    for (int b = 0; b < LOOK; ++b) {
        const bool live = !done;
        valid_mask |= live ? (1u << b) : 0u;
        tt[b] = fminf(fminf(D.tdist[0], fminf(D.tdist[1], D.tdist[2])), this_tmax);
        const int cell = (D.cur[0] * res + D.cur[1]) * res + D.cur[2];
        safe_cell = live ? cell : safe_cell;
        cellv[b] = safe_cell;
        const bool sx = (D.tdist[0] < D.tdist[1]) && (D.tdist[0] < D.tdist[2]);
        const bool sy = !sx && (D.tdist[1] < D.tdist[2]);
        const bool sz = !sx && !sy;
        const float nx = D.tdist[0] + D.delta[0], ny = D.tdist[1] + D.delta[1], nz = D.tdist[2] + D.delta[2];
        D.tdist[0] = (live && sx) ? nx : D.tdist[0];
        D.tdist[1] = (live && sy) ? ny : D.tdist[1];
        D.tdist[2] = (live && sz) ? nz : D.tdist[2];
        D.cur[0] += (live && sx) ? D.stp[0] : 0;
        D.cur[1] += (live && sy) ? D.stp[1] : 0;
        D.cur[2] += (live && sz) ? D.stp[2] : 0;
        const bool over = (sx & (D.cur[0] == D.ovf[0])) | (sy & (D.cur[1] == D.ovf[1])) | (sz & (D.cur[2] == D.ovf[2]));
        done = done || (live && over);
    }
    D.safe_cell = safe_cell;
    D.done = done;
    return valid_mask;
}

template <int LOOK>
CED_HD int load_batch(const uint8_t *__restrict__ grid, const int (&cellv)[LOOK], const AccelSpec &S, bool accel, const Dda &D,
                      int lvl, int res, uint8_t (&occ)[LOOK])
{
#pragma unroll
    for (int b = 0; b < LOOK; ++b) occ[b] = grid[cellv[b]];
    int radius = 0;
    if (accel) {
        const int c0 = D.done ? 0 : D.cur[0], c1 = D.done ? 0 : D.cur[1], c2 = D.done ? 0 : D.cur[2];
        radius = empty_radius(S, lvl, res, c0, c1, c2);
    }
    return radius;
}

struct MarchCursor {
    float t_last;
    int n = 0;
    bool continuous = false;
    bool has_skip = false;
    float skip_to = 0.0f;
    CED_HD void push_skip(float target)
    {
        skip_to = has_skip ? fmaxf(skip_to, target) : target;
        has_skip = true;
    }
    CED_HD void empty_cell(float t_trav)
    {
        push_skip(t_trav);
        continuous = false;
    }
    CED_HD void flush_skip(const GridSpec &G)
    {
        if (has_skip) { t_last = skip_march_lattice(G, t_last, skip_to); has_skip = false; }
    }
};

template <class Emit>
CED_HD bool emit_cell(const GridSpec &G, MarchCursor &C, float t_trav, Emit &emit)
{
    while (C.n < G.limit) {
        float t_next;
        if (G.step_size <= 0.0f) {
            t_next = t_trav;
        } else {
            const float dt = calc_dt(C.t_last, G.cone_angle, G.step_size, 1e10f);
            if (C.t_last + dt * 0.5f >= t_trav) break;
            t_next = C.t_last + dt;
        }
        emit(C.n, C.t_last, t_next);
        C.n += 1;
        C.continuous = true;
        C.t_last = t_next;
        if (t_next >= t_trav) break;
    }
    return C.n >= G.limit;
}

template <int LOOK, bool SINGLE, bool PHASED, class Idx, class Emit>
CED_HD int traverse_ray_frame(const GridSpec &G, const AccelSpec &S, bool start_coarse, const float (&o)[3],
                              const float (&d)[3], float near, float far, const float *__restrict__ ts_row,
                              const Idx *__restrict__ ti_row, const uint8_t *__restrict__ hit_row, Emit &&emit,
                              float &t_term)
{
    const float inv_d[3] = { 1.0f / d[0], 1.0f / d[1], 1.0f / d[2] };
    const int n_grids = SINGLE ? 1 : G.n_grids, res = G.res;
    const bool accel = S.bdist != nullptr;
    MarchCursor C{ near };
    for (int i = 0; i < 2 * n_grids - 1; ++i) {
        if (C.n >= G.limit) break;
        int lvl;
        float seg_a, seg_b;
        if (!decode_segment<SINGLE>(G, o, inv_d, ts_row, ti_row, hit_row, i, lvl, seg_a, seg_b)) continue;
        const float this_tmin = fmaxf(seg_a, near);
        const float this_tmax = fminf(seg_b, far);
        if (this_tmin >= this_tmax) continue;
        if (!C.continuous) C.push_skip(this_tmin);
        const float *ab = G.aabbs + 6 * lvl;
        bool coarse = accel && start_coarse;
        bool traced = false;
        float t_stop0 = 0.0f, cells0 = 0.0f;
        if (coarse) {
            if (coarse_advance(S, lvl, res, ab, o, d, this_tmin, this_tmax, t_stop0, cells0)) {
                C.continuous = false;
                continue;
            }
            traced = true;
        }
        CED_DIAG_TICK(1);
        Dda D;
#pragma unroll
        for (int a = 0; a < 3; ++a) dda_setup_axis(D, a, res, ab, o, d, inv_d, this_tmin, this_tmax);
        dda_begin(D, res);
        const uint8_t *grid = G.binaries + (int64_t)lvl * res * res * res;
        float t_c = this_tmin;
        bool last_empty = false;
        int radius = 0;
        while (!D.done) {
            if (coarse) {
                coarse = false;
                float t_stop = t_stop0, cells = cells0;
                if (traced) {
                    traced = false;
                } else if (coarse_advance(S, lvl, res, ab, o, d, t_c, this_tmax, t_stop, cells)) {
                    C.continuous = false;
                    break;
                }
                if (cells >= kMinJumpCells) {
                    CED_DIAG_TICK(3);
                    float last_event = t_c;
                    bool any = false;
#pragma unroll
                    for (int a = 0; a < 3; ++a) {
                        const int kcap = D.stp[a] > 0 ? D.ovf[a] - D.cur[a] : (D.stp[a] < 0 ? D.cur[a] - D.ovf[a] : 0);
                        if (kcap <= 0) continue;
                        float prev = 0.0f;
                        const int k = count_steps(D.tdist[a], D.delta[a], t_stop, kcap, prev);
                        if (k > 0) {
                            D.cur[a] += k * D.stp[a];
                            last_event = any ? fmaxf(last_event, prev) : prev;
                            any = true;
                            if (k == kcap) D.done = true;
                        }
                    }
                    if (any) {
                        C.continuous = false;
                        const float t_in = fminf(last_event, this_tmax);
                        C.push_skip(t_in);
                        t_c = t_in;
                    }
                    if (D.done) break;
                }
            }
            if constexpr (PHASED) {
                float tt[LOOK];
                unsigned valid_mask = 0, occ_mask = 0;
                do {
                    CED_DIAG_TICK(4);
                    int cellv[LOOK];
                    uint8_t occ[LOOK];
                    valid_mask = look_ahead<LOOK>(D, res, this_tmax, tt, cellv);
                    radius = load_batch<LOOK>(grid, cellv, S, accel, D, lvl, res, occ);
                    occ_mask = 0;
#pragma unroll
                    for (int b = 0; b < LOOK; ++b) occ_mask |= occ[b] ? (1u << b) : 0u;
                    occ_mask &= valid_mask;
                    last_empty = false;
#pragma unroll
                    for (int b = 0; b < LOOK; ++b) {
                        const bool before = (valid_mask >> b & 1u) && (occ_mask & ((2u << b) - 1u)) == 0u;
                        if (before) { C.empty_cell(tt[b]); last_empty = true; t_c = tt[b]; }
                    }
                    if (occ_mask) break;
                    coarse = last_empty && radius >= kCoarseRadius;
                } while (!D.done && !coarse);
                if (occ_mask) {
                    CED_DIAG_TICK(5);
                    for (int b = __builtin_ctz(occ_mask); b < LOOK; ++b) {
                        if (!(valid_mask >> b & 1u)) break;
                        float t_trav = tt[0];
#pragma unroll
                        for (int k = 1; k < LOOK; ++k) t_trav = b == k ? tt[k] : t_trav;
                        if (!(occ_mask >> b & 1u)) { C.empty_cell(t_trav); last_empty = true; t_c = t_trav; continue; }
                        last_empty = false;
                        C.flush_skip(G);
                        if (emit_cell(G, C, t_trav, emit)) { t_term = C.t_last; return C.n; }
                    }
                    coarse = last_empty && radius >= kCoarseRadius;
                }
            } else {
                do {
                    CED_DIAG_TICK(4);
                    float tt[LOOK];
                    int cellv[LOOK];
                    uint8_t occ[LOOK];
                    const unsigned valid_mask = look_ahead<LOOK>(D, res, this_tmax, tt, cellv);
                    radius = load_batch<LOOK>(grid, cellv, S, accel, D, lvl, res, occ);
                    last_empty = false;
#pragma unroll
                    for (int b = 0; b < LOOK; ++b) {
                        if (!(valid_mask >> b & 1u)) continue;
                        if (!occ[b]) { C.empty_cell(tt[b]); last_empty = true; t_c = tt[b]; continue; }
                        last_empty = false;
                        CED_DIAG_TICK(5);
                        C.flush_skip(G);
                        if (emit_cell(G, C, tt[b], emit)) { t_term = C.t_last; return C.n; }
                    }
                    coarse = last_empty && radius >= kCoarseRadius;
                } while (!D.done && !coarse);
            }
        }
    }
    t_term = C.t_last;
    return C.n;
}

template <class Emit>
CED_HD int traverse_ray(const GridSpec &G, const float (&o)[3], const float (&d)[3], float near, float far,
                        const float *__restrict__ ts_row, const int64_t *__restrict__ ti_row,
                        const uint8_t *__restrict__ hit_row, Emit &&emit, float &t_term)
{
    const float inv_d[3] = { 1.0f / d[0], 1.0f / d[1], 1.0f / d[2] };
    const int res = G.res;
    const AccelSpec none{ nullptr, 0, nullptr };
    MarchCursor C{ near };
    bool owed = false;
    float owed_to = 0.0f;
    for (int i = 0; i < 2 * G.n_grids - 1; ++i) {
        if (C.n >= G.limit) break;
        int lvl;
        float seg_a, seg_b;
        if (!decode_segment<false>(G, o, inv_d, ts_row, ti_row, hit_row, i, lvl, seg_a, seg_b)) continue;
        const float this_tmin = fmaxf(seg_a, near);
        const float this_tmax = fminf(seg_b, far);
        if (this_tmin >= this_tmax) continue;
        if (owed) { C.t_last = skip_march(C.t_last, owed_to, G.step_size, G.cone_angle); owed = false; }
        if (!C.continuous) C.t_last = skip_march(C.t_last, this_tmin, G.step_size, G.cone_angle);
        const float *ab = G.aabbs + 6 * lvl;
        Dda D;
#pragma unroll
        for (int a = 0; a < 3; ++a) dda_setup_axis(D, a, res, ab, o, d, inv_d, this_tmin, this_tmax);
        dda_begin(D, res);
        const uint8_t *grid = G.binaries + (int64_t)lvl * res * res * res;
        bool stop = false, has_pending = false;
        float pending = 0.0f;
        while (!D.done && !stop) {
            float tt[kLook];
            int cellv[kLook];
            uint8_t occ[kLook];
            const unsigned valid_mask = look_ahead<kLook>(D, res, this_tmax, tt, cellv);
            (void)load_batch<kLook>(grid, cellv, none, false, D, lvl, res, occ);
#pragma unroll
            for (int b = 0; b < kLook; ++b) {
                if (!(valid_mask >> b & 1u) || stop) continue;
                if (!occ[b]) {
                    pending = tt[b];
                    has_pending = true;
                    C.continuous = false;
                    continue;
                }
                if (has_pending) {
                    C.t_last = skip_march(C.t_last, pending, G.step_size, G.cone_angle);
                    has_pending = false;
                }
                stop = emit_cell(G, C, tt[b], emit);
            }
        }
        if (has_pending) { owed = true; owed_to = pending; }
    }
    if (owed) C.t_last = skip_march(C.t_last, owed_to, G.step_size, G.cone_angle);
    t_term = C.t_last;
    return C.n;
}

}
```

### include/cednerf_hip.h

```cpp
#ifndef CEDNERF_HIP_H
#define CEDNERF_HIP_H

#include <stddef.h>
#include <stdint.h>

#ifdef __cplusplus
extern "C" {
#endif

#define CED_MAX_LEVELS 16

#define CED_OK 0
#define CED_E_INVALID (-1)
#define CED_E_LAUNCH (-2)
#define CED_E_UNSUPPORTED (-3)

typedef struct ced_hash_desc {
    int32_t n_levels;
    int32_t table_dtype;
    int32_t temporal;
    int32_t reserved;
    float scale[CED_MAX_LEVELS];
    uint32_t res[CED_MAX_LEVELS];
    uint32_t offset[CED_MAX_LEVELS];
    uint32_t size[CED_MAX_LEVELS];
    uint32_t hashed[CED_MAX_LEVELS];
    const void *table;
    uint64_t total_entries;
} ced_hash_desc;

typedef struct ced_field_desc {
    float aabb[6];
    float moving_step;
    int32_t use_div_offsets;
    int32_t time_mode;
    int32_t mlp_precision;
    int32_t max_workgroups;
    const void *packed_weights;
    uint64_t packed_floats;
    ced_hash_desc hash;
} ced_field_desc;

int ced_version(void);
const char *ced_last_error_string(void);

int ced_set_option(const char *key, int value);

#define CED_MLP_F32 0
#define CED_MLP_F16X2 1
#define CED_MLP_F16 2
#define CED_MLP_F32_HEAD16X2 3

int64_t ced_packed_weight_floats(int use_div_offsets, int time_mode);

int ced_pack_field_weights(int use_div_offsets, int time_mode,
                           const float *m_w0, const float *m_w1, const float *m_w2, const float *m_w3,
                           const float *b_w0, const float *b_w1,
                           const float *h_w0, const float *h_w1, const float *h_w2,
                           float *out);

int64_t ced_packed_weight_words(int use_div_offsets, int time_mode, int mlp_precision);
int ced_pack_field_weights_half(int use_div_offsets, int time_mode, int mlp_precision,
                                const float *m_w0, const float *m_w1, const float *m_w2, const float *m_w3,
                                const float *b_w0, const float *b_w1,
                                const float *h_w0, const float *h_w1, const float *h_w2,
                                void *out);
int ced_pack_field_weights_half_for(int use_div_offsets, int time_mode, int mlp_precision, int table_dtype, int temporal,
                                    const float *m_w0, const float *m_w1, const float *m_w2, const float *m_w3,
                                    const float *b_w0, const float *b_w1,
                                    const float *h_w0, const float *h_w1, const float *h_w2,
                                    void *out);
int ced_pack_field_weights_mixed(int use_div_offsets, int time_mode,
                                 const float *m_w0, const float *m_w1, const float *m_w2, const float *m_w3,
                                 const float *b_w0, const float *b_w1,
                                 const float *h_w0, const float *h_w1, const float *h_w2,
                                 float *out);

int ced_ray_aabb_intersect(int64_t n_rays, const float *rays_o, const float *rays_d,
                           int32_t n_aabbs, const float *aabbs,
                           float near_plane, float far_plane, float miss_value,
                           float *t_mins, float *t_maxs, uint8_t *hits, void *stream);

int ced_sort_intersections(int64_t n_rays, int32_t n_grids, const float *t_mins, const float *t_maxs, float *t_sorted,
                           int64_t *t_indices, void *stream);

int ced_traverse_grids(int64_t n_rays, const float *rays_o, const float *rays_d,
                       const uint8_t *binaries, int32_t n_grids, int32_t res, const float *aabbs,
                       const float *near_planes, const float *far_planes,
                       float step_size, float cone_angle, int32_t limit, const uint8_t *rays_mask,
                       const float *t_sorted, const int64_t *t_indices, const uint8_t *hits,
                       int32_t mode, const int64_t *base,
                       int64_t *counts, float *t_starts, float *t_ends, int64_t *ray_indices,
                       float *termination_planes, int64_t *packed_info_out, void *stream);

int64_t ced_occupancy_accel_bytes(int32_t n_grids, int32_t res);
int ced_build_occupancy_accel(const uint8_t *binaries, int32_t n_grids, int32_t res, void *accel, int64_t accel_bytes,
                              void *stream);

int ced_host_build_occupancy_accel(const uint8_t *binaries_host, int32_t n_grids, int32_t res, uint8_t *accel_host);
int32_t ced_host_count_steps(float *x, float d, float tau, int32_t kcap, float *prev);
int ced_host_march_frame(int64_t n_rays, const float *rays_o, const float *rays_d, const uint8_t *binaries,
                         int32_t n_grids, int32_t res, const float *aabbs, const float *near_planes, float far_plane,
                         float step_size, float cone_angle, int32_t limit, const float *t_sorted,
                         const int64_t *t_indices, const uint8_t *hits, const uint8_t *accel_host, int32_t accel_mode,
                         int32_t use_lattice, int32_t walk, int32_t *counts, float *t_starts, float *t_ends,
                         float *t_term);

float ced_host_skip_march(float t_last, float target, float step_size, float cone_angle);

int ced_hash_encode(const ced_hash_desc *desc, int64_t n, const float *x, const float *t,
                    float *out, void *stream);

int ced_hash_encode_backward(const ced_hash_desc *desc, int64_t n, const float *x, const float *dy,
                             float *grad_table, float *dx, int32_t dx_scaled, void *stream);

int ced_hash_encode_backward_temporal(const ced_hash_desc *desc, int64_t n, const float *x, const float *t,
                                      const float *dy, float *grad_table, void *stream);

int ced_field_forward(const ced_field_desc *desc, int64_t n, const float *positions, const float *t,
                      const float *directions, float *rgb, float *sigma, float *geo, void *stream);

int ced_field_forward_rays(const ced_field_desc *desc, int64_t n, const int64_t *n_dev,
                           const float *rays_o, const float *rays_d,
                           const int64_t *ray_indices, const float *t_starts, const float *t_ends,
                           const float *timestamps, int32_t t_per_ray, int32_t want_rgb,
                           float *rgb, float *sigma, void *stream);

int ced_field_move(const ced_field_desc *desc, int64_t n, const float *positions, const float *t,
                   float *x_move, float *move, float *x_norm, uint8_t *selector, void *stream);

int ced_field_move_rays(const ced_field_desc *desc, int64_t n, const int64_t *n_dev,
                        const float *rays_o, const float *rays_d,
                        const int64_t *ray_indices, const float *t_starts, const float *t_ends,
                        const float *timestamps, int32_t t_per_ray, float *move, float *x_norm, void *stream);

int ced_field_move_inverse(const ced_field_desc *desc, int64_t n, const float *target, const float *t,
                           const float *init, int32_t max_iters, float tol, float *x, float *step,
                           int32_t *evals, void *stream);

int ced_field_track(const ced_field_desc *desc, int64_t n_points, int64_t n_times, const float *target,
                    const float *times, const float *init, int32_t max_iters, float tol, float *x,
                    float *step, int32_t *evals, void *stream);

int ced_field_move_jacobian(const ced_field_desc *desc, int64_t n, const float *positions, const float *t,
                            float *move, float *jac, void *stream);

int ced_field_move_inverse_newton(const ced_field_desc *desc, int64_t n, const float *target, const float *t,
                                  const float *init, int32_t max_iters, float tol, float *x, float *step,
                                  int32_t *evals, void *stream);

int ced_field_track_newton(const ced_field_desc *desc, int64_t n_points, int64_t n_times, const float *target,
                           const float *times, const float *init, int32_t max_iters, float tol, float *x,
                           float *step, int32_t *evals, void *stream);

int ced_field_velocity(const ced_field_desc *desc, int64_t n, const float *positions, const float *t,
                       float *velocity, float *det, uint8_t *valid, void *stream);

int ced_field_velocity_rays(const ced_field_desc *desc, int64_t n, const int64_t *n_dev,
                            const float *rays_o, const float *rays_d,
                            const int64_t *ray_indices, const float *t_starts, const float *t_ends,
                            const float *timestamps, int32_t t_per_ray, float *velocity, float *det, uint8_t *valid,
                            void *stream);

int ced_field_density_gradient(const ced_field_desc *desc, int64_t n, const float *positions, const float *t,
                               float *sigma, float *grad, float *dlog, float *dlog_canonical, void *stream);

int ced_field_density_gradient_rays(const ced_field_desc *desc, int64_t n, const int64_t *n_dev,
                                    const float *rays_o, const float *rays_d,
                                    const int64_t *ray_indices, const float *t_starts, const float *t_ends,
                                    const float *timestamps, int32_t t_per_ray, float *sigma, float *grad, float *dlog,
                                    float *dlog_canonical, void *stream);

#define CED_TIME_MAX_BINS 256
#define CED_TIME_MAX_TIMES 64
int ced_field_density_time_max(const ced_field_desc *desc, int64_t n, const float *positions, int32_t n_bins,
                               int32_t n_times, const float *times, float *out, void *stream);

int64_t ced_occ_time_slices_workspace_bytes(int32_t n_bins, int32_t levels, int32_t res);
int ced_occ_time_slices(int64_t n, const int64_t *cell_ids, const float *max_sigma, int32_t n_bins, float step_size,
                        float thre, int32_t levels, int32_t res, const uint8_t *union_binaries, int32_t dilate,
                        uint8_t *out, void *workspace, int64_t workspace_bytes, void *stream);

#define CED_LEVEL_SET_MAX_ITERS 64
int ced_surface_first_crossing(int64_t n_rays, const int64_t *packed_info, const float *t_starts, const float *t_ends,
                               const float *sigmas, float thresh, int64_t *k, float *lo, float *hi, void *stream);
int ced_field_level_set(const ced_field_desc *desc, int64_t n, const float *origins, const float *dirs, const float *lo,
                        const float *hi, const float *times, int32_t t_per_row, float thresh, int32_t max_iters, float tol,
                        float *t, float *x, float *sigma, float *width, int32_t *status, int32_t *evals, void *stream);

int ced_field_rgb(const ced_field_desc *desc, int64_t n, const float *dirs, const float *embedding,
                  int32_t apply_act, float *rgb, void *stream);

int ced_field_rgb_bcast(const ced_field_desc *desc, int64_t m, int32_t n_dirs, const float *dirs,
                        const float *embedding, int32_t apply_act, float *rgb, void *stream);

int64_t ced_bake_workspace_bytes(int64_t n);

int ced_bake_candidates(int32_t reso, const float *center_host, float radius, int64_t first_cell, int64_t n_cells,
                        const uint8_t *binaries, const float *aabbs, int32_t levels, int32_t grid_res,
                        int64_t capacity, int64_t *index, float *xyz, int64_t *count, void *workspace,
                        int64_t workspace_bytes, void *stream);

int ced_bake_select(int64_t n, const int64_t *index_in, const float *xyz_in, const float *sigma_in,
                    const float *embedding_in, float sigma_thresh, int64_t capacity, int64_t *index, float *xyz,
                    float *sigma, float *embedding, int64_t *count, void *workspace, int64_t workspace_bytes,
                    void *stream);

int64_t ced_mesh_workspace_bytes(int32_t reso);

int ced_mesh_vertices(int32_t reso, const float *center_host, float radius, const float *lattice, float thresh,
                      int64_t capacity, float *vertices, float *normals, int64_t *cube, int64_t *count,
                      void *workspace, int64_t workspace_bytes, void *stream);

int ced_mesh_faces(int32_t reso, const float *lattice, float thresh, const int64_t *cube, int64_t n_vertices,
                   int64_t capacity, int32_t *faces, int64_t *count, void *workspace, int64_t workspace_bytes,
                   void *stream);

int ced_render_weights(int64_t n_rays, const int64_t *packed_info, const float *t_starts,
                       const float *t_ends, const float *sigmas, const float *prefix_trans,
                       float *weights, float *trans, float *alphas, void *stream);

int ced_accumulate_along_rays(int64_t n_rays, const int64_t *packed_info, const float *weights,
                              const float *values, int32_t n_channels, float *out, void *stream);

int ced_reduce_along_rays(int64_t n_samples, const int64_t *ray_indices, const float *values, int32_t n_channels,
                          const float *weights, int32_t weight_channels, int64_t n_rays, int32_t mean, float *out,
                          int32_t *counts_workspace, void *stream);

int ced_visibility_mask(int64_t n_rays, const int64_t *packed_info, const float *t_starts,
                        const float *t_ends, const float *sigmas, float early_stop_eps, float alpha_thre,
                        uint8_t *mask, void *stream);

int ced_composite_prefix(int64_t n_rays, const int64_t *packed_info, const float *t_starts,
                         const float *t_ends, const float *sigmas, const float *rgbs,
                         float *rgb, float *opacity, float *depth, void *stream);

int ced_composite_backward(int64_t n_rays, const int64_t *packed_info, const float *t_starts,
                           const float *t_ends, const float *sigmas, const float *rgbs,
                           const float *d_color, const float *d_opacity, const float *d_depth,
                           float *d_sigmas, float *d_rgbs, void *stream);

int64_t ced_distortion_workspace_bytes(int64_t n_rays, int64_t n_samples, int32_t density);
int ced_distortion_loss(int64_t n_rays, int64_t n_samples, const int64_t *packed_info, const float *weights,
                        const float *t_starts, const float *t_ends, float *ray_loss, float *grad_weights,
                        void *workspace, float *loss, float *inv_norm, void *stream);
int ced_distortion_loss_density(int64_t n_rays, int64_t n_samples, const int64_t *packed_info, const float *sigmas,
                                const float *t_starts, const float *t_ends, float *ray_loss, float *d_sigmas,
                                void *workspace, float *loss, float *inv_norm, void *stream);

int64_t ced_ssim_workspace_bytes(int64_t n, int64_t c, int64_t h, int64_t w, int32_t win_size, int32_t levels);
int ced_ssim(int64_t n, int64_t c, int64_t h, int64_t w, const float *x, const int64_t *x_strides, const float *y,
             const int64_t *y_strides, double data_range, double k1, double k2, int32_t win_size, const float *win,
             int32_t levels, const float *weights, int32_t nonnegative, float *per_image, float *mean, double *mse,
             double *level_means, void *workspace, void *stream);

int ced_frame_to_rgb8(int32_t height, int32_t width, const float *rgb, int32_t flip_w, uint8_t *out, void *stream);
int ced_depth_to_u8(int32_t height, int32_t width, const float *depth, int32_t flip_w, uint8_t *out,
                    void *workspace, void *stream);

int ced_flow_to_rgb8(int32_t height, int32_t width, const float *flow, float max_mag, int32_t flip_w, uint8_t *out,
                     void *stream);

int ced_scatter_pixels(int64_t n_rows, const float *src_rgb, int32_t stride_rgb, const float *src_opacity,
                       int32_t stride_opacity, const float *src_depth, int32_t stride_depth, const int64_t *dest,
                       int64_t n_pixels, float *rgb, float *opacity, float *depth, uint8_t *rgb8, int32_t width,
                       int32_t flip_w, void *stream);

int ced_linear(int64_t n, const float *x, int32_t n_in, const float *w, int32_t w_rows, int32_t w_cols,
               int32_t transpose_w, int32_t n_out, int32_t relu, const float *mask, float *y, void *stream);

int64_t ced_weight_grad_workspace_bytes(int64_t n, int32_t n_out, int32_t n_in);
int ced_weight_grad(int64_t n, const float *x, int32_t n_in, const float *dy, int32_t n_out, float *dw,
                    void *workspace, int64_t workspace_bytes, void *stream);

int ced_composite_step(int64_t n_rays, const int64_t *packed_info, const float *t_starts,
                       const float *t_ends, const float *sigmas, const float *rgbs,
                       float *rgb, float *opacity, float *depth,
                       float opc_thres, int32_t n_samples_iter, uint8_t *ray_mask, int64_t *stats,
                       void *stream);

int ced_composite_test(int64_t n_alive, const float *sigmas, const float *rgbs, const float *t_start,
                       const float *t_end, const int64_t *pack_info, int64_t *alive_indices,
                       float T_threshold, float alpha_threshold,
                       float *opacity, float *depth, float *rgb, void *stream);

int ced_finalize_pixels(int64_t n_rays, const float *bkgd, float *rgb, const float *opacity,
                        float *depth, void *stream);


int ced_occ_cell_points(int64_t n, const int64_t *cell_indices, const float *noise, int32_t res,
                        const float *aabb_host, float *positions, void *stream);

int ced_occ_ema_update(int64_t n, const int64_t *cell_ids, const float *density, float step_size,
                       float ema_decay, float *occs, void *workspace, int64_t workspace_bytes, void *stream);


int ced_generate_rays_pinhole(int32_t width, int32_t height, float fx, float fy, float cx, float cy,
                              const float *c2w_host, int32_t opengl, float *origins, float *viewdirs,
                              float *directions, void *stream);

int ced_generate_rays_hypercam(int32_t width, int32_t height, const float *orientation_host,
                               const float *position_host, float focal_length, float principal_x, float principal_y,
                               float skew, float pixel_aspect_ratio, const float *radial3_host,
                               const float *tangential2_host, float *origins, float *viewdirs, void *stream);

#define CED_CAMERA_PINHOLE 0
#define CED_CAMERA_HYPERCAM 1
#define CED_PINHOLE_FLOATS 17
#define CED_HYPERCAM_FLOATS 22
#define CED_VIEW_PER_RAY 0
#define CED_VIEW_PER_STEP 1
#define CED_BKGD_WHITE 0
#define CED_BKGD_BLACK 1
#define CED_BKGD_RANDOM 2
int ced_sample_training_batch(int32_t camera_model, int32_t n_views, int32_t width, int32_t height, int32_t channels,
                              const uint8_t *images, const float *cameras, const float *view_timestamps,
                              int64_t num_rays, uint64_t seed, int64_t step, int32_t view_mode, int32_t bkgd_mode,
                              float *origins, float *viewdirs, float *pixels, float *timestamps, float *color_bkgd,
                              int32_t *indices, void *stream);

int64_t ced_importance_batch_workspace_bytes(int64_t n_cells, int64_t pool_size, int64_t num_cells);
int ced_sample_importance_batch(int32_t camera_model, int32_t n_views, int32_t width, int32_t height, int32_t channels,
                                const uint8_t *images, const float *cameras, const float *view_timestamps,
                                const float *weights, int32_t weights_subsampled, int64_t pool_size, int64_t num_cells,
                                uint64_t seed, int64_t step, int32_t bkgd_mode, float *origins, float *viewdirs,
                                float *pixels, float *timestamps, float *color_bkgd, int32_t *indices, uint32_t *min_key,
                                void *workspace, int64_t workspace_bytes, void *stream);

int ced_temporal_median_u8(int32_t n_cameras, int32_t n_frames, int32_t height, int32_t width, const uint8_t *images,
                           uint8_t *median, void *stream);
int ced_isg_weights(int32_t n_cameras, int32_t n_frames, int32_t height, int32_t width, const uint8_t *images,
                    const uint8_t *median, float gamma, float *weights, void *stream);
int ced_ist_weights(int32_t n_cameras, int32_t n_frames, int32_t height, int32_t width, const uint8_t *images,
                    float alpha, int32_t frame_shift, float *weights, void *stream);

typedef struct ced_frame_trace {
    int32_t capacity;
    int32_t n_iters;
    void **field_begin;
    void **field_end;
    int64_t *iter_alive;
    int64_t *iter_n_samples;
    int64_t *iter_samples;
    uint64_t *field_stamps;
} ced_frame_trace;

int64_t ced_wall_clock_khz(void);

int64_t ced_render_image_test_workspace_bytes(int64_t n_rays, int32_t n_grids, int32_t res, float cone_angle,
                                              int32_t max_samples);

int ced_render_image_test(const ced_field_desc *field, int64_t n_rays, const float *rays_o, const float *rays_d,
                          const uint8_t *binaries, int32_t n_grids, int32_t res, const float *aabbs, const void *accel,
                          float near_plane, float far_plane, float render_step_size, float cone_angle,
                          float early_stop_eps, int32_t max_samples,
                          const float *timestamps, int32_t t_per_ray, const float *bkgd,
                          float *rgb, float *opacity, float *depth,
                          void *workspace, int64_t workspace_bytes, int64_t *host_stats,
                          int64_t *total_samples_out, ced_frame_trace *trace, void *field_stream, void *stream);

int64_t ced_render_frames_test_workspace_bytes(int32_t n_frames, int64_t rays_per_frame, int32_t n_grids, int32_t res,
                                               float cone_angle, int32_t max_samples);
int ced_render_frames_test(const ced_field_desc *field, int32_t n_frames, int64_t rays_per_frame,
                           const float *rays_o, const float *rays_d, const uint8_t *binaries, int32_t n_grids,
                           int32_t res, const float *aabbs, const void *accel, float near_plane, float far_plane,
                           float render_step_size, float cone_angle, float early_stop_eps, int32_t max_samples,
                           const float *frame_times, const float *bkgd, float *rgb, float *opacity, float *depth,
                           void *workspace, int64_t workspace_bytes, int64_t *host_stats,
                           int64_t *total_samples_out, ced_frame_trace *trace, void *field_stream, void *stream);

typedef int (*ced_exchange_fn)(void *user, int64_t *counts, int32_t n_counts, int32_t iteration, void *stream);
typedef struct ced_shard_exchange {
    int64_t global_rays_per_frame;
    const int32_t *local_rays;
    int64_t *counts;
    ced_exchange_fn reduce;
    void *user;
} ced_shard_exchange;
int64_t ced_render_frames_test_sharded_workspace_bytes(int32_t n_frames, int64_t rays_per_frame,
                                                       int64_t global_rays_per_frame, int32_t n_grids, int32_t res,
                                                       float cone_angle, int32_t max_samples);
int32_t ced_render_frames_test_iterations(float cone_angle, int32_t max_samples);
int64_t ced_render_frames_test_host_bytes(float cone_angle, int32_t max_samples);
int ced_render_frames_test_sharded(const ced_field_desc *field, int32_t n_frames, int64_t rays_per_frame,
                                   const float *rays_o, const float *rays_d, const uint8_t *binaries, int32_t n_grids,
                                   int32_t res, const float *aabbs, const void *accel, float near_plane, float far_plane,
                                   float render_step_size, float cone_angle, float early_stop_eps, int32_t max_samples,
                                   const float *frame_times, const float *bkgd, float *rgb, float *opacity, float *depth,
                                   void *workspace, int64_t workspace_bytes, int64_t *host_stats,
                                   int64_t *total_samples_out, ced_frame_trace *trace, void *field_stream, void *stream,
                                   const ced_shard_exchange *exchange);

int64_t ced_render_image_workspace_bytes(int64_t n_rays, int64_t n_all);
int ced_render_image(const ced_field_desc *field, int64_t n_rays, const float *rays_o, const float *rays_d,
                     int64_t n_all, const int64_t *packed_info, const float *t_starts, const float *t_ends,
                     float early_stop_eps, float alpha_thre, const float *timestamps, int32_t t_per_ray,
                     const float *bkgd, float *rgb, float *opacity, float *depth, int32_t *kept, void *workspace,
                     int64_t workspace_bytes, int64_t *host_stats, int64_t *stats_out, void *field_stream, void *stream);
int ced_render_image_gather(int64_t n_rays, int64_t n_all, int64_t processed, const void *workspace,
                            int64_t workspace_bytes, const int64_t *ray_offsets, int64_t chunk_rays,
                            int64_t *ray_indices, float *t_starts, float *t_ends, float *sigmas, float *rgbs,
                            float *weights, float *trans, float *alphas, void *stream);

int ced_march_all(int64_t n_rays, const float *rays_o, const float *rays_d, const uint8_t *binaries, int32_t n_grids,
                  int32_t res, const float *aabbs, const void *accel, const float *near_planes, float far_plane,
                  float render_step_size, float cone_angle, const float *t_sorted, const int64_t *t_indices,
                  const uint8_t *hits, int32_t fill, int64_t *packed_info, float *t_starts, float *t_ends,
                  int64_t *ray_indices, int64_t capacity, int64_t *total, void *stream);

int ced_mlp_chain(int64_t n, int32_t n_layers, int32_t backward, const float *x, const int32_t *widths,
                  const float *const *weights, float *const *outs, const float *const *masks, int32_t relu_last,
                  void *stream);

int64_t ced_mlp_backward_dw_workspace_bytes(int64_t n, int32_t n_layers, const int32_t *widths);
int ced_mlp_backward_dw(int64_t n, int32_t n_layers, const float *dy, const int32_t *widths,
                        const float *const *weights, const float *const *acts, float *g0, float *dws, void *workspace,
                        int64_t workspace_bytes, void *stream);

int ced_train_inputs(int64_t n, const float *rays_o, const float *rays_d, const int64_t *ray_indices,
                     const float *t_starts, const float *t_ends, const float *timestamps, const float *positions,
                     const float *directions, float *pos_out, float *enc_out, float *sh_out, float *t_out, void *stream);
int ced_train_warp(int64_t n, const float *pos, const float *mo, int32_t mo_width, int32_t use_div_offsets,
                   float moving_step, const float *aabb_host, float *xn, float *move, float *selector, void *stream);
int ced_train_warp_backward(int64_t n, const float *pos, const float *mo, int32_t mo_width, int32_t use_div_offsets,
                            float moving_step, const float *aabb_host, const float *d_xn, const float *d_move,
                            float *d_mo, void *stream);
int ced_train_head_in(int64_t n, const float *bout, const float *sh, const float *selector, float *head_in,
                      float *sigma, void *stream);
int ced_train_head_in_backward(int64_t n, const float *bout, const float *selector, const float *d_head_in,
                               const float *d_sigma, float *d_bout, void *stream);

#ifdef __cplusplus
}
#endif
#endif
```

Before: 4.612 billion.

## Add conservative per-64-ray group clearance to skip empty-space marching

Adds kernels that compute, for each group of 64 adjacent rays, conservative bounds on origin and direction spread, then walk the occupancy distance field to find a shared distance along which the whole group is guaranteed empty. The march and cull kernels use this value as a starting hint for coarse_advance, and skip whole workgroups or waves when every group is clear for its full span. The aim is to cut per-ray empty-space traversal in the first march iteration. In exchange it adds two small kernels, extra scratch memory (carve now takes a frame count), and conservative-bound logic that must stay correct, plus host reference versions.

After: 4.678 billion (median of 6 runs). 1.4% higher.

```diff
diff --git a/ced_nerf_amd/_lib.py b/ced_nerf_amd/_lib.py
--- a/ced_nerf_amd/_lib.py
+++ b/ced_nerf_amd/_lib.py
@@ -78,6 +78,9 @@
     "ced_host_count_steps": (_i32, [C.POINTER(C.c_float), _f, _f, _i32, C.POINTER(C.c_float)]),
     "ced_host_march_frame": (C.c_int, [_i64, _vp, _vp, _vp, _i32, _i32, _vp, _vp, _f, _f, _f, _i32, _vp, _vp, _vp, _vp, _i32, _i32,
                                        _i32, _vp, _vp, _vp, _vp]),
+    "ced_host_march_frame_hinted": (C.c_int, [_i64, _vp, _vp, _vp, _i32, _i32, _vp, _vp, _f, _f, _f, _i32, _vp, _vp, _vp, _vp, _i32,
+                                              _i32, _i32, _vp, _vp, _vp, _vp, _vp]),
+    "ced_host_ray_group_clear": (C.c_int, [_i32, _i64, _vp, _vp, _vp, _i32, _i32, _vp, _vp, _i32, _f, _f, _vp]),
     "ced_hash_encode": (C.c_int, [C.POINTER(HashDesc), _i64, _vp, _vp, _vp, _vp]),
     "ced_hash_encode_backward": (C.c_int, [C.POINTER(HashDesc), _i64, _vp, _vp, _vp, _vp, _i32, _vp]),
     "ced_hash_encode_backward_temporal": (C.c_int, [C.POINTER(HashDesc), _i64, _vp, _vp, _vp, _vp, _vp]),
diff --git a/ced_nerf_amd/csrc/accel.hip b/ced_nerf_amd/csrc/accel.hip
--- a/ced_nerf_amd/csrc/accel.hip
+++ b/ced_nerf_amd/csrc/accel.hip
@@ -286,12 +286,12 @@
     return ced::count_steps(*x, d, tau, kcap, *prev);
 }
 
-extern "C" int ced_host_march_frame(int64_t n_rays, const float *rays_o, const float *rays_d, const uint8_t *binaries,
-                                    int32_t n_grids, int32_t res, const float *aabbs, const float *near_planes,
-                                    float far_plane, float step_size, float cone_angle, int32_t limit,
-                                    const float *t_sorted, const int64_t *t_indices, const uint8_t *hits,
-                                    const uint8_t *accel_host, int32_t accel_mode, int32_t use_lattice, int32_t walk,
-                                    int32_t *counts, float *t_starts, float *t_ends, float *t_term)
+static int host_march_frame(int64_t n_rays, const float *rays_o, const float *rays_d, const uint8_t *binaries,
+                            int32_t n_grids, int32_t res, const float *aabbs, const float *near_planes,
+                            float far_plane, float step_size, float cone_angle, int32_t limit,
+                            const float *t_sorted, const int64_t *t_indices, const uint8_t *hits,
+                            const uint8_t *accel_host, int32_t accel_mode, int32_t use_lattice, int32_t walk,
+                            const float *t_hint, int32_t *counts, float *t_starts, float *t_ends, float *t_term)
 {
     CED_REQUIRE(n_rays >= 0 && n_grids >= 1 && res >= 1 && limit >= 1, "host_march_frame: bad sizes");
     CED_REQUIRE(rays_o && rays_d && binaries && aabbs && near_planes && t_sorted && t_indices && hits && counts &&
@@ -313,15 +313,77 @@
         const int64_t *ti = t_indices + r * 2 * n_grids;
         const uint8_t *hr = hits + r * n_grids;
         const float near = near_planes[r];
+        const float hint = t_hint ? t_hint[r] : -__builtin_inff();
         float &tt = t_term[r];
         if (walk == 3)
             counts[r] = ced::traverse_ray(G, o, d, near, far_plane, ts, ti, hr, emit, tt);
         else if (n_grids == 1)
-            counts[r] = walk == 1 ? ced::traverse_ray_frame<ced::kFrameLook, true, true>(G, S, true, o, d, near, far_plane, ts, ti, hr, emit, tt)
-                                  : ced::traverse_ray_frame<ced::kFrameLook, true, false>(G, S, walk != 0, o, d, near, far_plane, ts, ti, hr, emit, tt);
+            counts[r] = walk == 1 ? ced::traverse_ray_frame<ced::kFrameLook, true, true>(G, S, true, o, d, near, far_plane, ts, ti, hr, emit, tt, hint)
+                                  : ced::traverse_ray_frame<ced::kFrameLook, true, false>(G, S, walk != 0, o, d, near, far_plane, ts, ti, hr, emit, tt, hint);
         else
-            counts[r] = walk == 1 ? ced::traverse_ray_frame<ced::kFrameLook, false, true>(G, S, true, o, d, near, far_plane, ts, ti, hr, emit, tt)
-                                  : ced::traverse_ray_frame<ced::kFrameLook, false, false>(G, S, walk != 0, o, d, near, far_plane, ts, ti, hr, emit, tt);
+            counts[r] = walk == 1 ? ced::traverse_ray_frame<ced::kFrameLook, false, true>(G, S, true, o, d, near, far_plane, ts, ti, hr, emit, tt, hint)
+                                  : ced::traverse_ray_frame<ced::kFrameLook, false, false>(G, S, walk != 0, o, d, near, far_plane, ts, ti, hr, emit, tt, hint);
     }
     return CED_OK;
 }
+
+extern "C" int ced_host_march_frame(int64_t n_rays, const float *rays_o, const float *rays_d, const uint8_t *binaries,
+                                    int32_t n_grids, int32_t res, const float *aabbs, const float *near_planes,
+                                    float far_plane, float step_size, float cone_angle, int32_t limit,
+                                    const float *t_sorted, const int64_t *t_indices, const uint8_t *hits,
+                                    const uint8_t *accel_host, int32_t accel_mode, int32_t use_lattice, int32_t walk,
+                                    int32_t *counts, float *t_starts, float *t_ends, float *t_term)
+{
+    return host_march_frame(n_rays, rays_o, rays_d, binaries, n_grids, res, aabbs, near_planes, far_plane, step_size, cone_angle,
+                            limit, t_sorted, t_indices, hits, accel_host, accel_mode, use_lattice, walk, nullptr, counts, t_starts,
+                            t_ends, t_term);
+}
+
+extern "C" int ced_host_march_frame_hinted(int64_t n_rays, const float *rays_o, const float *rays_d, const uint8_t *binaries,
+                                           int32_t n_grids, int32_t res, const float *aabbs, const float *near_planes,
+                                           float far_plane, float step_size, float cone_angle, int32_t limit,
+                                           const float *t_sorted, const int64_t *t_indices, const uint8_t *hits,
+                                           const uint8_t *accel_host, int32_t accel_mode, int32_t use_lattice, int32_t walk,
+                                           const float *t_hint, int32_t *counts, float *t_starts, float *t_ends,
+                                           float *t_term)
+{
+    CED_REQUIRE(t_hint != nullptr, "host_march_frame_hinted: null t_hint");
+    return host_march_frame(n_rays, rays_o, rays_d, binaries, n_grids, res, aabbs, near_planes, far_plane, step_size, cone_angle,
+                            limit, t_sorted, t_indices, hits, accel_host, accel_mode, use_lattice, walk, t_hint, counts, t_starts,
+                            t_ends, t_term);
+}
+
+extern "C" int ced_host_ray_group_clear(int32_t n_frames, int64_t rays_per_frame, const int32_t *local_rays,
+                                        const float *rays_o, const float *rays_d, int32_t n_grids, int32_t res,
+                                        const float *aabbs, const uint8_t *accel_host, int32_t accel_mode, float near_plane,
+                                        float far_plane, float *t_clear)
+{
+    CED_REQUIRE(n_frames >= 1 && rays_per_frame >= 0 && n_grids >= 1 && n_grids <= 8 && res >= 1, "host_ray_group_clear: bad sizes");
+    CED_REQUIRE(rays_o && rays_d && aabbs && accel_host && t_clear, "host_ray_group_clear: null pointer");
+    CED_REQUIRE(accel_mode == 1 || accel_mode == 2, "host_ray_group_clear: accel_mode 1 (bricks), 2 (cells)");
+    const ced::AccelSpec S = ced::accel_view(accel_host, n_grids, res, accel_mode == 2);
+    const int64_t gpf = (rays_per_frame + ced::kGroupRays - 1) / ced::kGroupRays;
+    const float inf = __builtin_inff();
+    for (int64_t G = 0; G < (int64_t)n_frames * gpf; ++G) {
+        const int64_t f = G / gpf, k0 = (G % gpf) * ced::kGroupRays;
+        const int64_t count = local_rays ? local_rays[f] : rays_per_frame;
+        if (k0 >= count) { t_clear[G] = inf; continue; }
+        const int members = (int)((count - k0 < ced::kGroupRays) ? count - k0 : ced::kGroupRays);
+        const int64_t rc = f * rays_per_frame + k0 + ced::group_reference(members);
+        ced::RayGroupBounds B;
+        for (int a = 0; a < 3; ++a) { B.oc[a] = rays_o[3 * rc + a]; B.dc[a] = rays_d[3 * rc + a]; }
+        float v[6 + 2 * ced::kGroupMaxLevels], lim[2 * ced::kGroupMaxLevels];
+        for (float &x : v) x = -inf;
+        bool bad = false;
+        for (int64_t r = f * rays_per_frame + k0; r < f * rays_per_frame + k0 + members; ++r) {
+            const float o[3] = { rays_o[3 * r], rays_o[3 * r + 1], rays_o[3 * r + 2] };
+            const float d[3] = { rays_d[3 * r], rays_d[3 * r + 1], rays_d[3 * r + 2] };
+            ced::group_member(o, d, B.oc, B.dc, n_grids, aabbs, v, bad);
+        }
+        for (int a = 0; a < 3; ++a) { B.dev_o[a] = v[a]; B.dev_d[a] = v[3 + a]; }
+        for (int l = 0; l < n_grids; ++l) { lim[2 * l] = -v[6 + 2 * l]; lim[2 * l + 1] = v[7 + 2 * l]; }
+        if (bad) B.dev_o[0] = inf;
+        t_clear[G] = ced::group_clear(S, n_grids, res, aabbs, B, lim, near_plane, far_plane);
+    }
+    return CED_OK;
+}
diff --git a/ced_nerf_amd/csrc/frame.hip b/ced_nerf_amd/csrc/frame.hip
--- a/ced_nerf_amd/csrc/frame.hip
+++ b/ced_nerf_amd/csrc/frame.hip
@@ -82,7 +82,97 @@
     int32_t *ray_idx;
     int32_t *packed;
     int32_t *cand;
+    const float *t_clear;
+    int groups_per_frame;
 };
+
+constexpr int kGroupThreads = 256;
+static_assert(kGroupMaxLevels == kMaxGrids, "group_member's per-level limits");
+static_assert(kSlotAlign % kGroupRays == 0 && kGroupRays == 64, "a wave's slots of the first iteration are one group");
+template <int NV>
+__global__ __launch_bounds__(kGroupThreads) void ray_group_bounds_kernel(
+    int n_frames, int rays_per_frame, int groups_per_frame, const int32_t *__restrict__ local_rays,
+    const float *__restrict__ rays_o, const float *__restrict__ rays_d, int m, const float *__restrict__ aabbs,
+    RayGroupBounds *__restrict__ bounds, float *__restrict__ limits)
+{
+    static_assert(NV == 8 || NV == 16 || NV == 32, "6 + 2 m values, padded");
+    const int lane = threadIdx.x & 63;
+    const int64_t n_groups = (int64_t)n_frames * groups_per_frame;
+    const float inf = __builtin_inff();
+    int mine = 0;
+#pragma unroll
+    for (int s = 0; (NV >> s) > 1; ++s) mine += ((lane >> s) & 1) * (NV >> (s + 1));
+    for (int64_t g = (int64_t)blockIdx.x * (kGroupThreads / 64) + (threadIdx.x >> 6); g < n_groups;
+         g += (int64_t)gridDim.x * (kGroupThreads / 64)) {
+        const int f = (int)(g / groups_per_frame);
+        const int k0 = (int)(g % groups_per_frame) * kGroupRays;
+        const int count = local_rays ? local_rays[f] : rays_per_frame;
+        const int members = count - k0 < kGroupRays ? count - k0 : kGroupRays;
+        if (members <= 0) continue;
+        const int64_t r = (int64_t)f * rays_per_frame + k0 + (lane < members ? lane : 0);
+        const float o[3] = { rays_o[3 * r], rays_o[3 * r + 1], rays_o[3 * r + 2] };
+        const float d[3] = { rays_d[3 * r], rays_d[3 * r + 1], rays_d[3 * r + 2] };
+        const int ref = group_reference(members);
+        const float oc[3] = { __shfl(o[0], ref, 64), __shfl(o[1], ref, 64), __shfl(o[2], ref, 64) };
+        const float dc[3] = { __shfl(d[0], ref, 64), __shfl(d[1], ref, 64), __shfl(d[2], ref, 64) };
+        float v[6 + 2 * kMaxGrids > NV ? 6 + 2 * kMaxGrids : NV];
+#pragma unroll
+        for (float &x : v) x = -inf;
+        bool bad = false;
+        if (lane < members) group_member(o, d, oc, dc, m, aabbs, v, bad);
+#pragma unroll
+        for (int s = 0; (NV >> s) > 1; ++s) {
+            const int half = NV >> (s + 1);
+            const bool up = (lane >> s) & 1;
+#pragma unroll
+            for (int k = 0; k < half; ++k) {
+                const float keep = up ? v[k + half] : v[k], send = up ? v[k] : v[k + half];
+                v[k] = fmaxf(keep, __shfl_xor(send, 1 << s, 64));
+            }
+        }
+#pragma unroll
+        for (int off = NV; off < 64; off <<= 1) v[0] = fmaxf(v[0], __shfl_xor(v[0], off, 64));
+        bad = __any(bad);
+        float *B = reinterpret_cast<float *>(bounds + g);
+        if (lane == ref) {
+#pragma unroll
+            for (int a = 0; a < 3; ++a) { B[a] = oc[a]; B[3 + a] = dc[a]; }
+        }
+        if (lane < NV) {
+            if (mine < 6) B[6 + mine] = (bad && mine == 0) ? inf : v[0];
+            else if (mine < 6 + 2 * m) limits[g * 2 * m + (mine - 6)] = (mine & 1) ? v[0] : -v[0];
+        }
+    }
+}
+
+__global__ __launch_bounds__(kGroupThreads) void ray_group_clear_kernel(
+    int n_frames, int rays_per_frame, int groups_per_frame, const int32_t *__restrict__ local_rays, AccelSpec S, int m, int res,
+    const float *__restrict__ aabbs, const RayGroupBounds *__restrict__ bounds, const float *__restrict__ limits,
+    float near_plane, float far_plane, float *__restrict__ t_clear)
+{
+    const int64_t g = (int64_t)blockIdx.x * kGroupThreads + threadIdx.x;
+    if (g >= (int64_t)n_frames * groups_per_frame) return;
+    const int count = local_rays ? local_rays[g / groups_per_frame] : rays_per_frame;
+    const bool empty = (int)(g % groups_per_frame) * kGroupRays >= count;
+    const RayGroupBounds B = bounds[g];
+    t_clear[g] = empty ? __builtin_inff() : group_clear(S, m, res, aabbs, B, limits + g * 2 * m, near_plane, far_plane);
+}
+
+template <int kWaves>
+__device__ __forceinline__ bool workgroup_clearance(const MarchArgs &A, const IterPlan &P, int f, int64_t s0, int wave, float &t_own)
+{
+    const int idx0 = (int)(s0 - P.slot_base[f]);
+    const float *row = A.t_clear + (int64_t)f * A.groups_per_frame + (idx0 >> 6);
+    bool all_clear = true;
+    t_own = 0.0f;
+#pragma unroll
+    for (int w = 0; w < kWaves; ++w) {
+        const float tc = idx0 + 64 * w < P.count[f] ? row[w] : __builtin_inff();
+        all_clear = all_clear && tc == __builtin_inff();
+        t_own = w == wave ? tc : t_own;
+    }
+    return all_clear;
+}
 
 constexpr int kCullThreads = 256;
 static_assert(kSlotAlign % kCullThreads == 0, "a culling workgroup's slots belong to one frame");
@@ -98,8 +188,18 @@
         const int64_t idx = s0 + threadIdx.x - P.slot_base[f];
         const bool active = idx < P.count[f];
         const int64_t r = (int64_t)f * A.rays_per_frame + (active ? idx : 0);
+        float t_hint = 0.0f;
+        if (A.t_clear) {
+            const bool all_clear = workgroup_clearance<kCullThreads / 64>(A, P, f, s0, __builtin_amdgcn_readfirstlane(threadIdx.x >> 6), t_hint);
+            if (all_clear) {
+                if (active) { A.packed[2 * r] = 0; A.packed[2 * r + 1] = 0; }
+                continue;
+            }
+        }
         bool cand = false;
-        if (active) {
+        if (active && t_hint == __builtin_inff()) {
+            A.packed[2 * r] = 0; A.packed[2 * r + 1] = 0;
+        } else if (active) {
             float o[3], d[3];
 #pragma unroll
             for (int a = 0; a < 3; ++a) { o[a] = A.rays_o[3 * r + a]; d[a] = A.rays_d[3 * r + a]; }
@@ -115,7 +215,7 @@
                 const float t0 = fmaxf(seg_a, near), t1 = fminf(seg_b, A.far_plane);
                 if (t0 >= t1) continue;
                 float t_stop, cells;
-                cand = !coarse_advance(A.accel, lvl, res, A.grid.aabbs + 6 * lvl, o, d, t0, t1, t_stop, cells);
+                cand = !coarse_advance(A.accel, lvl, res, A.grid.aabbs + 6 * lvl, o, d, t0, t1, t_stop, cells, t_hint);
             }
             if (!cand) { A.packed[2 * r] = 0; A.packed[2 * r + 1] = 0; }
         }
@@ -140,10 +240,14 @@
         int f = 0;
         bool active;
         int64_t r = 0;
+        float t_hint = 0.0f;
         if constexpr (CAND) {
             const int64_t slot = s0 + wave * kCandLanes + lane;
             active = lane < kCandLanes && slot < total;
-            if (active) { r = A.cand[slot]; f = (int)(r / A.rays_per_frame); }
+            if (active) {
+                r = A.cand[slot]; f = (int)(r / A.rays_per_frame);
+                if (A.t_clear) t_hint = A.t_clear[(int64_t)f * A.groups_per_frame + (r - (int64_t)f * A.rays_per_frame) / kGroupRays];
+            }
         } else {
             f = frame_of_slot(P, A.n_frames, s0);
             if (f < 0) continue;
@@ -151,6 +255,19 @@
             active = idx < P.count[f];
             const int64_t first = (int64_t)f * A.rays_per_frame;
             r = active ? (A.alive ? (int64_t)A.alive[first + idx] : first + idx) : 0;
+            if constexpr (FIRST) {
+                if (A.t_clear) {
+                    const bool all_clear = workgroup_clearance<kWaves>(A, P, f, s0, __builtin_amdgcn_readfirstlane(wave), t_hint);
+                    if (all_clear) {
+                        if (active) { A.packed[2 * r] = 0; A.packed[2 * r + 1] = 0; }
+                        continue;
+                    }
+                    if (t_hint == __builtin_inff()) {
+                        if (active) { A.packed[2 * r] = 0; A.packed[2 * r + 1] = 0; }
+                        active = false;
+                    }
+                }
+            }
         }
         const int limit = P.limit[f];
         GridSpec grid = A.grid;
@@ -168,7 +285,7 @@
             const int n = traverse_ray_frame<kFrameLook, SINGLE, FIRST>(
                 grid, A.accel, FIRST, o, d, near, A.far_plane,
                 SINGLE ? nullptr : A.t_sorted + r * 2 * m, SINGLE ? (const uint8_t *)nullptr : A.t_indices + r * 2 * m,
-                SINGLE ? nullptr : A.hits + r * m, emit, t_term);
+                SINGLE ? nullptr : A.hits + r * m, emit, t_term, t_hint);
             if constexpr (decltype(first)::value) A.near_planes[r] = t_term;
             return n;
         };
@@ -246,6 +363,9 @@
     float *t0, *t1; int32_t *ridx; float *sigma, *rgbs;
     uint8_t *accel;
     float *sh_ray;
+    float *group_clear;
+    RayGroupBounds *group_bounds;
+    float *group_limits;
     size_t bytes;
 };
 
@@ -262,8 +382,12 @@
     return per * n_frames;
 }
 
-static FrameWorkspace carve(void *base, int64_t n, int m, int64_t cap, int max_iters, int res, bool per_ray_times = false)
-{
+static inline int64_t groups_of(int64_t rays_per_frame) { return (rays_per_frame + kGroupRays - 1) / kGroupRays; }
+
+static FrameWorkspace carve(void *base, int n_frames, int64_t rays_per_frame, int m, int64_t cap, int max_iters, int res,
+                            bool per_ray_times = false)
+{
+    const int64_t n = (int64_t)n_frames * rays_per_frame, groups = (int64_t)n_frames * groups_of(rays_per_frame);
     FrameWorkspace w{};
     Carver c{ (char *)base };
     w.t_sorted = c.take<float>((size_t)n * 2 * m);
@@ -284,6 +408,9 @@
     const int64_t nbk = (res + kBrick - 1) / kBrick;
     w.accel = c.take<uint8_t>((size_t)(2 * m * nbk * nbk * nbk));
     w.sh_ray = c.take<float>((size_t)n * 3);
+    w.group_clear = c.take<float>((size_t)groups);
+    w.group_bounds = c.take<RayGroupBounds>((size_t)groups);
+    w.group_limits = c.take<float>((size_t)groups * 2 * m);
     w.bytes = c.off;
     return w;
 }
@@ -337,7 +464,7 @@
     const int64_t cap = sample_capacity(c.n_frames, c.rays_per_frame, min_samples, c.xch ? c.xch->global_rays_per_frame : 0);
     CED_REQUIRE(cap < (1ll << 31) - 64, "%s: too many samples per iteration for 32-bit sample indices", c.who);
     const int max_iters = max_iterations(c.max_samples, min_samples);
-    FrameWorkspace W = carve(c.workspace, n_rays, c.n_grids, cap, max_iters, c.res, c.frame_times != nullptr);
+    FrameWorkspace W = carve(c.workspace, c.n_frames, c.rays_per_frame, c.n_grids, cap, max_iters, c.res, c.frame_times != nullptr);
     CED_REQUIRE((int64_t)W.bytes <= c.workspace_bytes, "%s: workspace too small (%lld < %lld bytes)", c.who,
                 (long long)c.workspace_bytes, (long long)W.bytes);
     if (c.xch) {
@@ -365,6 +492,21 @@
         if (rc) return rc;
         acc = AccelSpec{ W.accel, nb, nullptr };
     }
+    const int gpf = (int)groups_of(c.rays_per_frame);
+    const bool clear_groups = acc.bdist && c.near_plane >= 0.0f;
+    if (clear_groups) {
+        const int64_t n_groups = (int64_t)c.n_frames * gpf;
+        const int32_t *local = c.xch ? c.xch->local_rays : nullptr;
+        int64_t agrid = (n_groups + kGroupThreads / 64 - 1) / (kGroupThreads / 64);
+        if (agrid > 16384) agrid = 16384;
+        const auto bounds_kernel = c.n_grids == 1 ? ray_group_bounds_kernel<8>
+                                   : (c.n_grids <= 5 ? ray_group_bounds_kernel<16> : ray_group_bounds_kernel<32>);
+        hipLaunchKernelGGL(bounds_kernel, dim3((unsigned)agrid), dim3(kGroupThreads), 0, stream, c.n_frames,
+                           (int)c.rays_per_frame, gpf, local, c.rays_o, c.rays_d, (int)c.n_grids, c.aabbs, W.group_bounds, W.group_limits);
+        hipLaunchKernelGGL(ray_group_clear_kernel, dim3((unsigned)((n_groups + kGroupThreads - 1) / kGroupThreads)), dim3(kGroupThreads),
+                           0, stream, c.n_frames, (int)c.rays_per_frame, gpf, local, acc, (int)c.n_grids, (int)c.res, c.aabbs,
+                           W.group_bounds, W.group_limits, c.near_plane, c.far_plane, W.group_clear);
+    }
     const bool use_lattice = c.cone_angle == 0.0f && c.step_size > 0.0f && c.near_plane >= 0.0f;
     if (use_lattice) build_lattice(c.near_plane, c.step_size, reinterpret_cast<float *>(c.host_stats + kHostLatticeWord));
     FrameLoop L{ ScheduleArgs{ W.plans, -1, c.n_frames, (int)c.rays_per_frame, min_samples, (int)c.max_samples,
@@ -392,7 +534,7 @@
         MarchArgs M{ c.rays_o, c.rays_d,
                      GridSpec{ c.binaries, c.aabbs, c.n_grids, c.res, c.step_size, c.cone_angle, 0, use_lattice ? W.lattice : nullptr },
                      acc, W.near, c.far_plane, cur_list, c.n_frames, (int)c.rays_per_frame, W.t_sorted, W.t_indices, W.hits,
-                     W.t0, W.t1, W.ridx, W.packed, W.alive_b };
+                     W.t0, W.t1, W.ridx, W.packed, W.alive_b, (it == 0 && clear_groups) ? W.group_clear : nullptr, gpf };
         int64_t mgrid = (slot_bound + kMarchThreads - 1) / kMarchThreads;
         if (mgrid > 8192) mgrid = 8192;
         const dim3 mblk(kMarchThreads);
@@ -499,7 +641,7 @@
 {
     if (n_rays < 0 || n_grids < 1 || n_grids > ced::kMaxGrids || res < 1 || res > 1024 || max_samples < 0) return -1;
     const int ms = ced::min_samples_of(cone_angle);
-    return (int64_t)ced::carve(nullptr, n_rays, n_grids, n_rays * ms, ced::max_iterations(max_samples, ms), res).bytes;
+    return (int64_t)ced::carve(nullptr, 1, n_rays, n_grids, n_rays * ms, ced::max_iterations(max_samples, ms), res).bytes;
 }
 
 extern "C" int ced_render_image_test(const ced_field_desc *field, int64_t n_rays, const float *rays_o,
@@ -557,9 +699,8 @@
     if (n_frames < 1 || n_frames > ced::kMaxFrames || rays_per_frame < 0 || global_rays_per_frame < rays_per_frame ||
         n_grids < 1 || n_grids > ced::kMaxGrids || res < 1 || res > 1024 || max_samples < 0)
         return -1;
-    const int64_t n_rays = (int64_t)n_frames * rays_per_frame;
     const int ms = ced::min_samples_of(cone_angle);
-    return (int64_t)ced::carve(nullptr, n_rays, n_grids, ced::sample_capacity(n_frames, rays_per_frame, ms, global_rays_per_frame),
+    return (int64_t)ced::carve(nullptr, n_frames, rays_per_frame, n_grids, ced::sample_capacity(n_frames, rays_per_frame, ms, global_rays_per_frame),
                                ced::max_iterations(max_samples, ms), res, true).bytes;
 }
 
diff --git a/ced_nerf_amd/csrc/march_accel.hpp b/ced_nerf_amd/csrc/march_accel.hpp
--- a/ced_nerf_amd/csrc/march_accel.hpp
+++ b/ced_nerf_amd/csrc/march_accel.hpp
@@ -98,7 +98,8 @@
 }
 
 CED_HD bool coarse_advance(const AccelSpec &S, int lvl, int res, const float *__restrict__ ab, const float (&o)[3],
-                           const float (&d)[3], float t_from, float t_to, float &t_stop, float &cells_skipped)
+                           const float (&d)[3], float t_from, float t_to, float &t_stop, float &cells_skipped,
+                           float t_probe = -__builtin_inff())
 {
     const float resf = (float)res;
     float sc[3], g = 0.0f;
@@ -111,7 +112,8 @@
     cells_skipped = 0.0f;
     if (!(g > 0.0f) || !(g < 3.0e38f) || !(t_to - t_from < 3.0e38f)) return false;
     const float inv_g = 1.0f / g;
-    float t = t_from;
+    float t = t_probe > 0.0f ? fmaxf(t_from, t_probe) : t_from;
+    if (t >= t_to) return true;
     for (int guard = 0; guard < 8192; ++guard) {
         CED_DIAG_TICK(2);
         int c[3];
@@ -124,6 +126,90 @@
     }
     t_stop = t_from;
     return false;
+}
+
+constexpr int kGroupRays = 64;
+constexpr int kGroupMaxLevels = 8;
+constexpr float kClearRel = 1.0f / 1048576.0f;
+constexpr float kClearAbs = 0.0625f;
+constexpr float kClearMinCells = 1.0f;
+
+struct RayGroupBounds {
+    float oc[3], dc[3], dev_o[3], dev_d[3];
+};
+
+CED_HD bool finite3(const float (&v)[3])
+{
+    return fabsf(v[0]) < __builtin_inff() && fabsf(v[1]) < __builtin_inff() && fabsf(v[2]) < __builtin_inff();
+}
+
+CED_HD int group_reference(int members) { return members * 9 / 16; }
+
+CED_HD void group_member(const float (&o)[3], const float (&d)[3], const float (&oc)[3], const float (&dc)[3], int n_grids,
+                         const float *__restrict__ aabbs, float *v, bool &bad)
+{
+    bad = bad || !finite3(o) || !finite3(d);
+    const float inv_d[3] = { 1.0f / d[0], 1.0f / d[1], 1.0f / d[2] };
+#pragma unroll
+    for (int a = 0; a < 3; ++a) {
+        v[a] = fmaxf(v[a], fabsf(o[a] - oc[a]));
+        v[3 + a] = fmaxf(v[3 + a], fabsf(d[a] - dc[a]));
+    }
+#pragma unroll
+    for (int l = 0; l < kGroupMaxLevels; ++l) {
+        float t0, t1;
+        if (l >= n_grids || !slab_test(o, inv_d, aabbs + 6 * l, t0, t1)) continue;
+        v[6 + 2 * l] = fmaxf(v[6 + 2 * l], -t0);
+        v[7 + 2 * l] = fmaxf(v[7 + 2 * l], t1);
+    }
+}
+
+CED_HD float group_clear_level(const AccelSpec &S, int lvl, int res, const float *__restrict__ ab, const RayGroupBounds &B,
+                               float t_lo, float t_hi)
+{
+    if (!(t_lo < t_hi)) return __builtin_inff();
+    const float resf = (float)res;
+    float sc[3], slope[3], base[3], per_t[3], g = 0.0f;
+#pragma unroll
+    for (int a = 0; a < 3; ++a) {
+        sc[a] = resf / (ab[3 + a] - ab[a]);
+        const float reach = fabsf(B.dc[a]) + B.dev_d[a];
+        slope[a] = sc[a] * reach * (1.0f + kClearRel);
+        base[a] = sc[a] * (B.dev_o[a] + kClearRel * (fabsf(B.oc[a]) + B.dev_o[a] + fmaxf(fabsf(ab[a]), fabsf(ab[3 + a])))) + kClearAbs;
+        per_t[a] = sc[a] * (B.dev_d[a] + kClearRel * reach);
+        g = fmaxf(g, slope[a]);
+    }
+    if (!(g > 0.0f) || !(g < 3.0e38f) || !(t_hi < 3.0e38f) || !(base[0] + base[1] + base[2] < 3.0e38f)) return t_lo;
+    float t = t_lo;
+    for (int guard = 0; guard < 8192; ++guard) {
+        int c[3];
+#pragma unroll
+        for (int a = 0; a < 3; ++a)
+            c[a] = clampi((int)fminf(fmaxf((B.oc[a] + B.dc[a] * t - ab[a]) * sc[a], -1.0f), resf), 0, res - 1);
+        const float room = (float)(empty_radius(S, lvl, res, c[0], c[1], c[2]) - 3);
+        float adv = __builtin_inff();
+#pragma unroll
+        for (int a = 0; a < 3; ++a) {
+            const float left = room - (base[a] + per_t[a] * t);
+            if (slope[a] > 0.0f) adv = fminf(adv, left / slope[a]);
+            else if (!(left >= 0.0f)) adv = -1.0f;
+        }
+        if (!(adv * g >= kClearMinCells)) return t;
+        t += adv;
+        if (t >= t_hi) return __builtin_inff();
+    }
+    return t;
+}
+
+CED_HD float group_clear(const AccelSpec &S, int n_grids, int res, const float *__restrict__ aabbs, const RayGroupBounds &B,
+                         const float *__restrict__ lim, float near, float far)
+{
+    if (!(near >= 0.0f)) return 0.0f;
+    if (!(finite3(B.oc) && finite3(B.dc) && finite3(B.dev_o) && finite3(B.dev_d))) return 0.0f;
+    float t_clear = __builtin_inff();
+    for (int lvl = 0; lvl < n_grids; ++lvl)
+        t_clear = fminf(t_clear, group_clear_level(S, lvl, res, aabbs + 6 * lvl, B, fmaxf(lim[2 * lvl], near), fminf(lim[2 * lvl + 1], far)));
+    return t_clear;
 }
 
 struct Dda {
@@ -254,7 +340,7 @@
 CED_HD int traverse_ray_frame(const GridSpec &G, const AccelSpec &S, bool start_coarse, const float (&o)[3],
                               const float (&d)[3], float near, float far, const float *__restrict__ ts_row,
                               const Idx *__restrict__ ti_row, const uint8_t *__restrict__ hit_row, Emit &&emit,
-                              float &t_term)
+                              float &t_term, float t_hint = -__builtin_inff())
 {
     const float inv_d[3] = { 1.0f / d[0], 1.0f / d[1], 1.0f / d[2] };
     const int n_grids = SINGLE ? 1 : G.n_grids, res = G.res;
@@ -274,7 +360,7 @@
         bool traced = false;
         float t_stop0 = 0.0f, cells0 = 0.0f;
         if (coarse) {
-            if (coarse_advance(S, lvl, res, ab, o, d, this_tmin, this_tmax, t_stop0, cells0)) {
+            if (coarse_advance(S, lvl, res, ab, o, d, this_tmin, this_tmax, t_stop0, cells0, t_hint)) {
                 C.continuous = false;
                 continue;
             }
diff --git a/include/cednerf_hip.h b/include/cednerf_hip.h
--- a/include/cednerf_hip.h
+++ b/include/cednerf_hip.h
@@ -105,6 +105,17 @@
                          const int64_t *t_indices, const uint8_t *hits, const uint8_t *accel_host, int32_t accel_mode,
                          int32_t use_lattice, int32_t walk, int32_t *counts, float *t_starts, float *t_ends,
                          float *t_term);
+
+int ced_host_ray_group_clear(int32_t n_frames, int64_t rays_per_frame, const int32_t *local_rays, const float *rays_o,
+                             const float *rays_d, int32_t n_grids, int32_t res, const float *aabbs,
+                             const uint8_t *accel_host, int32_t accel_mode, float near_plane, float far_plane,
+                             float *t_clear);
+int ced_host_march_frame_hinted(int64_t n_rays, const float *rays_o, const float *rays_d, const uint8_t *binaries,
+                                int32_t n_grids, int32_t res, const float *aabbs, const float *near_planes,
+                                float far_plane, float step_size, float cone_angle, int32_t limit, const float *t_sorted,
+                                const int64_t *t_indices, const uint8_t *hits, const uint8_t *accel_host,
+                                int32_t accel_mode, int32_t use_lattice, int32_t walk, const float *t_hint,
+                                int32_t *counts, float *t_starts, float *t_ends, float *t_term);
 
 float ced_host_skip_march(float t_last, float target, float step_size, float cone_angle);
 
```
